# DakeQQ/Voice-Activity-Detection-VAD-ONNX

Measured on NVIDIA B200. Metric: RTFx (audio-hours/sec), higher is better.
Workload: dtype f32

## Files before the change

### include/vadx.h

```cpp
#ifndef VADX_H_
#define VADX_H_

#include <stddef.h>
#include <stdint.h>

#ifdef __cplusplus
extern "C" {
#endif

#define VADX_ABI_VERSION 1

enum {
  VADX_OK = 0,
  VADX_EINVAL = -1,
  VADX_ENODEVICE = -2,
  VADX_ECUDA = -3,
  VADX_EMISSING = -4,
  VADX_ENOMEM = -5
};

enum { VADX_DT_I16 = 0, VADX_DT_F32 = 1, VADX_DT_I32 = 2 };
enum { VADX_ACT_NONE = 0, VADX_ACT_RELU = 1, VADX_ACT_SIGMOID = 2, VADX_ACT_SOFTMAX = 3,
       VADX_ACT_LOG = 4, VADX_ACT_LOG_CLAMP = 5, VADX_ACT_RES_FIRST = 16 };
enum { VADX_FLOOR_CLAMP = 0, VADX_FLOOR_ADD = 1 };
enum { VADX_PREEMPH_NONE = 0, VADX_PREEMPH_ZERO_HISTORY = 1, VADX_PREEMPH_KEEP_FIRST = 2 };

int vadx_abi_version(void);
const char* vadx_last_error(void);
int vadx_device_count(void);
uint64_t vadx_launch_count(void);

enum {
  VADX_STAGE_PREP = 0,
  VADX_STAGE_STFT = 1,
  VADX_STAGE_MEL = 2,
  VADX_STAGE_LINEAR = 3,
  VADX_STAGE_MEMORY = 4,
  VADX_STAGE_HEAD = 5,
  VADX_STAGE_POSTPROC = 6,
  VADX_STAGE_COUNT = 7
};
int vadx_profile_enable(int on);
int vadx_profile_collect(double* ms, uint64_t* calls, int n_stages);
typedef struct vadx_kernel_stat {
  const char* name;
  double ms;
  uint64_t calls;
  double bytes;
  double flops;
} vadx_kernel_stat;
int vadx_profile_collect_kernels(vadx_kernel_stat* out, int capacity, int* n_out);


int vadx_prep_audio(const void* d_audio, int in_dtype, int64_t n_streams, int64_t n_samples,
                    int64_t in_stride, float scale, int remove_dc, int preemph_mode, float preemph,
                    int64_t pad_left, float* d_out, int64_t out_stride, void* stream);

int vadx_stft_power_f32(const float* d_sig, int64_t sig_stride, int64_t n_streams, int n_frames, int hop,
                        int n_taps, const float* d_basis, int ld_basis, int n_bins, float* d_power,
                        int64_t ld_power, void* stream);

int vadx_stft_tc_supported(int n_taps, int n_bins);
int vadx_pack_stft_basis_tc(const float* h_basis, int ld_basis, int n_taps, int n_bins, double preemph, double scale,
                            void* h_img, size_t img_capacity, size_t* img_bytes);
int vadx_stft_power_tc_i16(const int16_t* d_audio, int64_t in_stride, int64_t n_samples, int64_t n_streams,
                           int n_frames, int hop, int n_taps, const void* d_img, int n_bins, float* d_power,
                           int64_t ld_power, void* stream);
int vadx_pack_stft_dc_tc(const float* h_basis, int ld_basis, int n_taps, int n_bins, double preemph, double scale,
                         int64_t n_samples, int hop, int pad_left, int n_frames, float* h_tables, size_t capacity_floats,
                         size_t* n_floats, int* n_edge_lo, int* t_edge_hi);
int vadx_stream_mean_i16(const int16_t* d_audio, int64_t in_stride, int64_t n_samples, int64_t n_streams,
                         float* d_mean_frac, int32_t* d_mean_int, void* stream);
int vadx_stft_power_tc_i16_ex(const int16_t* d_audio, int64_t in_stride, int64_t n_samples, int64_t n_streams,
                              int n_frames, int hop, int n_taps, const void* d_img, int n_bins, float* d_power,
                              int64_t ld_power, int pad_left, const float* d_mean_frac, const int32_t* d_mean_int,
                              const float* d_dc_tables, int n_edge_lo, int t_edge_hi, float power_scale,
                              int operand_format, void* stream);
enum { VADX_TC_FMT_BF16 = 0, VADX_TC_FMT_F16 = 1 };
int vadx_pack_stft_basis_tc_fmt(const float* h_basis, int ld_basis, int n_taps, int n_bins, double preemph, double scale,
                                int operand_format, void* h_img, size_t img_capacity, size_t* img_bytes);

int vadx_mel_log_f32(const float* d_power, int64_t ld_power, int64_t n_rows, int n_bins, int n_mels,
                     const int32_t* d_start, const int32_t* d_len, const float* d_w, int max_len,
                     int floor_mode, float floor_value, float* d_out, int64_t ld_out, void* stream);

int vadx_linear_f32(const float* d_x, int64_t ldx, const float* d_wt, int ldw, const float* d_bias,
                    const float* d_residual, int64_t ldr, float* d_y, int64_t ldy, int64_t n_rows, int n_in,
                    int n_out, int act, void* stream);

int vadx_tc_supported(int n_in, int n_out);
int vadx_pack_weight_tc(const float* h_w, int n_out, int n_in, void* h_img, size_t img_capacity, size_t* img_bytes);
int vadx_linear_tc_f32(const float* d_x, int64_t ldx, const void* d_wimg, const float* d_bias,
                       const float* d_residual, int64_t ldr, float* d_y, int64_t ldy, int64_t n_rows, int n_in,
                       int n_out, int act, void* stream);

int vadx_depthwise_conv1d_f32(const float* d_x, int64_t ldx, const float* d_w, int kernel, int stride, int dilation,
                              int pad, float* d_y, int64_t ldy, int64_t n_streams, int t_in, int t_out,
                              int n_channels, void* stream);

int vadx_linear_head_tc_f32(const float* d_x, int64_t ldx, const void* d_wimg, const float* d_bias, int64_t n_rows,
                            int n_in, int n_out, int act, const float* d_head_w, float head_bias, float* d_head_out,
                            void* stream);

int vadx_fsmn_memory_f32(const float* d_p, int64_t ldp, const float* d_wl, int n_back, int stride_back,
                         const float* d_wr, int n_ahead, int stride_ahead, const float* d_residual,
                         int64_t ldr, float* d_out, int64_t ldo, int64_t n_streams, int n_frames,
                         int n_channels, const float* d_cache_in, float* d_cache_out, void* stream);

size_t vadx_fc2_memory_stages_stream_bytes(int n_in, int n_frames);
int vadx_fc2_memory_stages_supported(int n_in, int n_out, int n_frames, int n_back, int stride_back, int n_ahead,
                                     int stride_ahead);
int vadx_linear_tc_stream_stages_f32(const float* d_x, const void* d_wimg, const float* d_bias, void* d_himg,
                                     int64_t n_rows, int rows_per_stream, int n_in, int n_out, int act, void* stream);
int vadx_fc2_memory_stages_f32(const void* d_himg, int n_in, const void* d_wimg, const float* d_bias, int act,
                               const float* d_wl, int n_back, const float* d_wr, int n_ahead, const float* d_residual,
                               float* d_out, int64_t n_streams, int n_frames, void* stream);

int vadx_lfr_cmvn_f32(const float* d_mel, int64_t ld_mel, const float* d_mean, const float* d_var, float* d_out,
                      int64_t ld_out, int64_t n_streams, int n_frames, int n_mels, int lfr_m, int lfr_n, void* stream);

int vadx_softmax_class0_f32(const float* d_logits, int64_t ld, int64_t n_rows, int n_classes, float* d_p0,
                            void* stream);

int vadx_frame_energy_log10_f32(const float* d_sig, int64_t sig_stride, int64_t offset, int64_t n_streams, int win,
                                int hop, int n_energy, int n_frames, float scale, float eps, float* d_out,
                                void* stream);

int vadx_fsmn_gate(const float* d_p_sil, const float* d_power_dB, const float* d_noise_avg,
                   float one_minus_speech_threshold, float speech_2_noise_ratio, int64_t n_streams, int n_frames,
                   uint8_t* d_score, float* d_noisy_dB, void* stream);

int vadx_lookahead_hysteresis(const void* d_in, int mode, int64_t ld_in, int64_t n_streams, int n_frames,
                              int look_backward, double speaking_score, double silence_score, int is_final,
                              uint8_t* d_silence_state, int32_t* d_n_saved, uint8_t* d_saved, int64_t ld_saved,
                              float* d_noise_avg, const float* d_noisy_dB, float snr_threshold, void* stream);

int vadx_fsmn_gate_hysteresis_windows(const float* d_p_sil, const float* d_power_dB, int64_t n_streams, int n_windows,
                                      int n_frames, float one_minus_speech_threshold, float speech_2_noise_ratio,
                                      int look_backward, double speaking_score, double silence_score, uint8_t* d_score,
                                      float* d_noisy_dB, float* d_noise_in, uint8_t* d_silence_state, int32_t* d_n_saved,
                                      uint8_t* d_saved, int64_t ld_saved, float* d_noise_avg, float snr_threshold,
                                      void* stream);

int vadx_gather_windows_i16(const int16_t* d_in, int64_t stream_stride, int64_t n_streams, int n_windows, int64_t window_stride,
                            int64_t n_samples, int16_t* d_out, void* stream);

int vadx_runs_to_segments(const uint8_t* d_silence_flags, int64_t ld, const int32_t* d_n_flags, int64_t n_streams,
                          int32_t* d_seg_count, int32_t* d_segments, int max_segments, void* stream);

int vadx_stft_mag_compact_f32(const float* d_y, int64_t ldy, int64_t n_windows, int rows_per_window, int n_frames,
                              int n_bins, float* d_mag, void* stream);
int vadx_reflect_window_f32(const float* d_x, int64_t in_stride, int64_t n_streams, int n_in, int pad, float* d_out,
                            void* stream);
int vadx_reflect_windows_f32(const float* d_x, int64_t in_stride, int64_t n_streams, int n_windows, int64_t window_step,
                             int n_in, int pad, float* d_out, void* stream);
int vadx_sqrt_inplace_f32(float* d_p, int64_t n, void* stream);
int vadx_affine_f32(const float* d_x, float a, float b, float* d_y, int64_t n, void* stream);
int vadx_lstm_cell_f32(const float* d_gates, const float* d_c_in, float* d_h_out, float* d_c_out, float* d_h_relu,
                       int64_t n_streams, int hidden, void* stream);

int vadx_silero_lstm_windows_f32(const float* d_gates_in, const float* d_wt_hh, int ldw, const float* d_state_in,
                                 float* d_state_out, const float* d_head_w, float head_bias, float* d_probs,
                                 int64_t n_streams, int n_windows, int hidden, void* stream);

int vadx_silero_timestamps(const float* d_probs, int64_t ld, const int32_t* d_n_windows, const int64_t* d_n_samples,
                           int64_t n_streams, double threshold, double neg_threshold, double min_speech_samples,
                           double max_speech_samples, double min_silence_samples,
                           double min_silence_samples_at_max_speech, int window, int use_max_poss_sil,
                           int32_t* d_seg_count, int64_t* d_segments, int max_segments, void* stream);

int vadx_stft_complex_f32(const float* d_sig, int64_t sig_stride, int64_t n_streams, int n_frames, int hop, int n_taps,
                          const float* d_basis, int ld_basis, int n_bins, float* d_out, int64_t ld_out, void* stream);
int vadx_permute4_f32(const float* d_in, float* d_out, int64_t n0, int64_t n1, int64_t n2, int64_t n3, int p0, int p1,
                      int p2, int p3, void* stream);
int vadx_layernorm_f32(const float* d_x, int64_t n_rows, int row_len, const float* d_w, const float* d_b, float eps,
                       float* d_out, void* stream);
int vadx_layernorm_perm_f32(const float* d_x, int64_t n_rows, int n1, int n2, int n3, int q0, int q1, int q2, const float* d_w,
                            const float* d_b, int w_out_order, float eps, float* d_out, int64_t out_stride, int pad, void* stream);
int vadx_ceps_cmul_t_f32(const float* d_q, const float* d_spec, float* d_out, int64_t n_blocks, int n_channels, int n_ceps,
                         void* stream);
int vadx_add_transposed_f32(const float* d_a, int64_t a_block_stride, const float* d_t, float* d_out, int64_t n_blocks, int n_bins,
                            int n_channels, void* stream);
int vadx_cfb_front_supported(int n_in, int n_channels, int n_bins);
int vadx_cfb_front_f32(const float* d_x, int64_t n_blocks, int n_bins, int n_in, int n_channels, const float* d_ln0_w,
                       const float* d_ln0_b, const float* d_wg, const float* d_bg, const float* d_wi, const float* d_bi,
                       const float* d_ln1_w, const float* d_ln1_b, const float* d_ln2_w, const float* d_ln2_b, float eps,
                       float* d_col, float* d_z, void* stream);
int vadx_lstm_seq_f32(const float* d_x, int64_t x_outer, int64_t x_inner, int64_t x_step, float* d_y, int64_t y_outer,
                      int64_t y_inner, int64_t y_step, const float* d_w_ih, const float* d_w_hh, const float* d_b_ih,
                      const float* d_b_hh, int64_t n_seq, int n_inner, int seq_len, int n_in, int hidden, int reverse,
                      void* stream);
int vadx_lstm_recurrence_supported(int hidden);
int vadx_lstm_recurrence_f32(const float* d_gates_in, int64_t g_outer, int64_t g_inner, int64_t g_step, float* d_y,
                             int64_t y_outer, int64_t y_inner, int64_t y_step, const float* d_w_hh_perm, int64_t n_seq,
                             int n_inner, int seq_len, int hidden, int reverse, void* stream);
int vadx_ew2_f32(int op, const float* d_a, int64_t lda, const float* d_b, int64_t ldb, float* d_out, int64_t ldo,
                 float* d_out2, int64_t ldo2, int64_t n_rows, int n_cols, float scalar, void* stream);
int vadx_ceps_cmul_f32(const float* d_q, const float* d_p, float* d_out, int64_t n_rows, int n_channels, void* stream);
int vadx_im2col_f3_f32(const float* d_x, float* d_out, int64_t n_blocks, int n_bins, int n_channels, void* stream);
int vadx_alpha_x4_f32(const float* d_near_ri, const float* d_far_ri, int64_t n_streams, int n_frames, int n_bins, int k,
                      float w1_far, float w1_mix, float b1, const float* d_w2, float b2, float* d_x4, float* d_alpha,
                      void* stream);
int vadx_alpha_x4_const_f32(const float* d_near_ri, const float* d_pow_far, const float* d_far_comp, int t_max,
                            int64_t n_streams, int n_frames, int n_bins, int k, float w1_far, float w1_mix, float b1,
                            const float* d_w2, float b2, float* d_x4, float* d_alpha, void* stream);
int vadx_istft_ola_f32(const float* d_frames, int64_t ld, int64_t n_streams, int n_frames, int n_fft, int hop,
                       const float* d_wsum_inv, int n_out, float* d_y, int64_t ldy, void* stream);

int64_t vadx_ingest_out_frames(int64_t n_frames_in, int in_rate, int out_rate);
int vadx_ingest_pcm16(const int16_t* d_pcm, int64_t in_stride, const int64_t* d_n_in, int64_t n_streams,
                      int64_t n_frames_in, int n_channels, int in_rate, int out_rate, int16_t* d_out,
                      int64_t out_stride, int64_t* d_n_out, void* stream);

int64_t vadx_resample_out_len(int64_t n_in, double scale);
int vadx_resample_linear_f32(const float* d_in, int64_t in_stride, int64_t n_in, int64_t n_streams, double scale,
                             float* d_out, int64_t out_stride, int64_t out_offset, void* stream);

typedef struct {
  int32_t smooth_window;
  float threshold;
  int32_t min_speech_frame;
  int32_t max_speech_frame;
  int32_t min_silence_frame;
  int32_t merge_silence_frame;
  int32_t extend_speech_frame;
} vadx_post_cfg;
int vadx_postprocess_frames(const float* d_probs, int64_t ld_probs, const int32_t* d_n_frames,
                            int64_t n_streams, int n_frames, const vadx_post_cfg* cfg, int8_t* d_decisions,
                            int32_t* d_seg_count, int32_t* d_segments, int max_segments, void* stream);

typedef struct {
  int32_t smooth_window;
  float threshold;
  int32_t pad_start_frame;
  int32_t min_speech_frame;
  int32_t max_speech_frame;
  int32_t min_silence_frame;
} vadx_stream_post_cfg;
int vadx_stream_post_state_words(int smooth_window);
int vadx_stream_postprocess(const float* d_probs, int64_t ld_probs, const int32_t* d_n_frames, int64_t n_streams,
                            int n_frames, const vadx_stream_post_cfg* cfg, int32_t* d_state, int32_t* d_seg_count,
                            int32_t* d_segments, int max_segments, int32_t* d_open, void* stream);

#define VADX_SERVE_START 0
#define VADX_SERVE_END 1
#define VADX_SERVE_END_OF_STREAM 2
#define VADX_SERVE_ERR_RANGE 1
#define VADX_SERVE_ERR_SHORT 2
int vadx_stream_serve_zero_tail(int16_t* d_chunk, int64_t ld_chunk, const int32_t* d_n_samples, int64_t n_slots,
                                int chunk_samples, int frame_len, void* stream);
int vadx_stream_serve_step(const float* d_probs, int64_t ld_probs, int n_frames, const int32_t* d_n_samples,
                           const uint8_t* d_last, int64_t n_slots, int chunk_samples, int frame_len, int frame_hop,
                           const vadx_stream_post_cfg* cfg, int32_t* d_state, const float* d_caches_in,
                           float* d_caches_out, int n_cache_blocks, int64_t cache_row, int32_t* d_frames,
                           int32_t* d_events, int32_t* d_header, int32_t* h_events, int32_t* h_header, void* d_scratch,
                           size_t scratch_bytes, size_t* scratch_needed, void* stream);

int vadx_silero_serve_load(const int16_t* d_chunk, const int32_t* d_n_samples, int64_t n_slots, int windows_per_tick,
                           float* d_x, void* stream);
int vadx_silero_serve_step(const float* d_probs, int64_t ld_probs, const int32_t* d_n_samples, const uint8_t* d_last,
                           int64_t n_slots, int windows_per_tick, double threshold, double min_silence_samples,
                           int32_t* d_state, float* d_x, const float* d_state_in, float* d_state_out,
                           int32_t* d_windows, int32_t* d_events, int32_t* d_header, int32_t* h_events,
                           int32_t* h_header, void* d_scratch, size_t scratch_bytes, size_t* scratch_needed,
                           void* stream);

typedef struct vadx_model vadx_model;

int vadx_create(const char* kind, const int32_t* hparams, int n_hparams, vadx_model** out);
void vadx_destroy(vadx_model* m);

int vadx_set_tensor(vadx_model* m, const char* name, const void* h_data, int dtype, const int64_t* dims,
                    int n_dims);
int vadx_set_scalar(vadx_model* m, const char* name, double value);

int vadx_workspace_bytes(const vadx_model* m, int64_t n_streams, int64_t n_samples, size_t* out_bytes);
int vadx_output_frames(const vadx_model* m, int64_t n_samples, int32_t* out_frames);

int vadx_forward(vadx_model* m, const void* const* d_inputs, void* const* d_outputs, void* const* d_state,
                 int64_t n_streams, int64_t n_samples, void* d_workspace, size_t workspace_bytes,
                 void* stream);

#ifdef __cplusplus
}
#endif
#endif
```

### voice-activity-detection-vad-onnx_b200/csrc/model.cu

```cuda
#include "model.hpp"

struct FireRedHP : FrontendGeom {
  int idim, R, M, H, P, N1, S1, N2, S2, odim;
  int frames(int64_t L) const { return L < n_taps() ? 0 : (int)(1 + (L - n_taps()) / hop); }
};

static int firered_hp(const vadx_model* m, FireRedHP* h) {
  VADX_REQUIRE(m->hp.size() == 14, "firered: expected 14 hyper-parameters, got %zu", m->hp.size());
  const int32_t* v = m->hp.data();
  *h = FireRedHP{{v[10], v[11], v[12], v[13]}, v[0], v[1], v[2], v[3], v[4], v[5], v[6], v[7], v[8], v[9]};
  VADX_REQUIRE(h->idim == h->n_mels, "firered: idim (%d) must equal n_mels (%d)", h->idim, h->n_mels);
  VADX_REQUIRE(h->R >= 1 && h->M >= 1 && h->H >= 1 && h->P >= 1 && h->N1 >= 1 && h->S1 >= 1 && h->N2 >= 0 &&
                   h->odim >= 1 && h->odim <= 8 && h->hop >= 1 && h->n_fft >= 2,
               "firered: hyper-parameter out of range");
  return VADX_OK;
}

static Frontend firered_frontend(const vadx_model* m, const FireRedHP& h) {
  return Frontend{h, (int)m->scalar("derived.bins_used", (double)h.n_bins()), 0, 1.0f, false, VADX_PREEMPH_ZERO_HISTORY,
                  VADX_TC_FMT_F16, VADX_FLOOR_CLAMP, (float)m->scalar("frontend.log_floor", 1e-7), frontend_rate_scale(m),
                  false};
}

int firered_finalize(vadx_model* m) {
  FireRedHP h;
  VADX_TRY(firered_hp(m, &h));
  int bins_used = 1;
  {
    const HostTensor* ms = m->find("frontend.mel_start");
    const HostTensor* ml = m->find("frontend.mel_len");
    if (ms && ml && ms->dtype == VADX_DT_I32 && ml->dtype == VADX_DT_I32 && ms->numel() == h.n_mels && ml->numel() == h.n_mels) {
      const int32_t* a = reinterpret_cast<const int32_t*>(ms->bytes.data());
      const int32_t* b = reinterpret_cast<const int32_t*>(ml->bytes.data());
      for (int i = 0; i < h.n_mels; ++i) bins_used = std::max(bins_used, a[i] + b[i]);
    } else {
      bins_used = h.n_bins();
    }
    bins_used = std::min(bins_used, h.n_bins());
    m->scalars["derived.bins_used"] = bins_used;
  }
  VADX_TRY(firered_frontend(m, h).finalize(m));
  VADX_TRY(m->upload_linear("dfsmn.fc1.0.weight", h.H, h.idim));
  VADX_TRY(m->upload_raw("dfsmn.fc1.0.bias", h.H, VADX_DT_F32));
  VADX_TRY(m->upload_linear("dfsmn.fc2.0.weight", h.P, h.H));
  VADX_TRY(m->upload_raw("dfsmn.fc2.0.bias", h.P, VADX_DT_F32));
  auto memory = [&](const std::string& pre) -> int {
    VADX_TRY(m->upload_raw(pre + "lookback_filter.weight", (int64_t)h.P * h.N1, VADX_DT_F32));
    if (h.N2 > 0) VADX_TRY(m->upload_raw(pre + "lookahead_filter.weight", (int64_t)h.P * h.N2, VADX_DT_F32));
    return VADX_OK;
  };
  VADX_TRY(memory("dfsmn.fsmn1."));
  for (int i = 0; i < h.R - 1; ++i) {
    std::string pre = "dfsmn.fsmns." + std::to_string(i) + ".";
    VADX_TRY(m->upload_linear(pre + "fc1.0.weight", h.H, h.P));
    VADX_TRY(m->upload_raw(pre + "fc1.0.bias", h.H, VADX_DT_F32));
    VADX_TRY(m->upload_linear(pre + "fc2.weight", h.P, h.H));
    VADX_TRY(memory(pre + "fsmn."));
  }
  VADX_TRY(m->upload_linear("dfsmn.dnns.0.weight", h.H, h.P));
  VADX_TRY(m->upload_raw("dfsmn.dnns.0.bias", h.H, VADX_DT_F32));
  for (int j = 1; j < h.M; ++j) {
    std::string n = "dfsmn.dnns." + std::to_string(2 * j);
    VADX_TRY(m->upload_linear(n + ".weight", h.H, h.H));
    VADX_TRY(m->upload_raw(n + ".bias", h.H, VADX_DT_F32));
  }
  VADX_TRY(m->upload_linear("out.weight", h.odim, h.H));
  VADX_TRY(m->upload_raw("out.weight", (int64_t)h.odim * h.H, VADX_DT_F32));
  VADX_TRY(m->upload_raw("out.bias", h.odim, VADX_DT_F32));
  return VADX_OK;
}

int firered_check(const vadx_model* m) {
  FireRedHP h;
  return firered_hp(m, &h);
}
int firered_frames(const vadx_model* m, int64_t n_samples, int32_t* out) {
  FireRedHP h;
  VADX_TRY(firered_hp(m, &h));
  const double sc = frontend_rate_scale(m);
  *out = h.frames(sc == 1.0 ? n_samples : vadx_resample_out_len(n_samples, sc));
  return VADX_OK;
}

static int64_t firered_slab(const vadx_model* m, int64_t S) {
  int64_t slab = (int64_t)m->scalar("engine.slab_streams", 0.0);
  if (slab <= 0 || slab > S) slab = S;
  return slab;
}

int firered_run(vadx_model* m, bool dry, const void* const* in, void* const* out, void* const* state, int64_t S_all,
                int64_t L, void* ws_ptr, size_t ws_bytes, size_t* need, cudaStream_t st) {
  FireRedHP h;
  VADX_TRY(firered_hp(m, &h));
  const int16_t* d_audio_all = dry ? nullptr : static_cast<const int16_t*>(in[0]);
  float* d_probs_all = dry ? nullptr : static_cast<float*>(out[0]);
  const float* cin_all = (!dry && state && state[0]) ? static_cast<const float*>(state[0]) : nullptr;
  float* cout_all = (!dry && state && state[0]) ? static_cast<float*>(state[1]) : nullptr;
  if (cin_all) {
    VADX_REQUIRE(h.N2 == 0, "firered: the streaming graph has no look-ahead taps (N2 must be 0, got %d)", h.N2);
    VADX_REQUIRE(cout_all && cout_all != cin_all, "firered: streaming needs a caches_out buffer distinct from caches_in");
  }
  const int64_t cache_stream = (int64_t)h.P * (h.N1 - 1) * h.S1;
  const int64_t cache_layer = S_all * cache_stream;
  const Frontend fe = firered_frontend(m, h);
  const double rate_scale = fe.rate_scale;
  const int64_t L16 = rate_scale == 1.0 ? L : vadx_resample_out_len(L, rate_scale);
  const int T = h.frames(L16);
  VADX_REQUIRE(T >= 1, "firered: %lld samples are shorter than one %d-sample frame", (long long)L16, h.n_taps());
  const int64_t slab = firered_slab(m, S_all);
  const int64_t slab_rows = slab * T;
  const int64_t Lp = round_up(std::max(L, L16), 4);
  Workspace ws(ws_ptr, ws_bytes, dry);
  float* sig = ws.take<float>(slab * Lp);
  float* sig2 = rate_scale == 1.0 ? nullptr : ws.take<float>(slab * Lp);
  float* power = ws.take<float>(slab_rows * h.ld_power());
  float* feat = ws.take<float>(slab_rows * h.n_mels);
  const int64_t bufH_floats = std::max<int64_t>(round_up(slab_rows, 128) * h.H,
                                                (h.H % 64) == 0 ? slab * (int64_t)(fc2_memory_stages_stream_bytes(h.H, T) / 4) : 0);
  float* bufH = ws.take<float>(bufH_floats);
  float* bufH2 = h.M > 1 ? ws.take<float>(slab_rows * h.H) : nullptr;
  float* bufP = ws.take<float>(slab_rows * h.P);
  float* memA0 = ws.take<float>(slab_rows * h.P);
  float* memB0 = ws.take<float>(slab_rows * h.P);
  if (need) *need = ws.off;
  if (dry) return VADX_OK;
  if (ws.off > ws_bytes) {
    set_error("firered: workspace of %zu bytes is smaller than the %zu needed", ws_bytes, ws.off);
    return VADX_ENOMEM;
  }

  for (int64_t s0 = 0; s0 < S_all; s0 += slab) {
    const int64_t S = std::min(slab, S_all - s0);
    const int64_t rows = S * T;
    const int16_t* d_audio = d_audio_all + s0 * L;
    float* d_probs = d_probs_all + s0 * (int64_t)h.odim * T;
    const float* cin = cin_all ? cin_all + s0 * cache_stream : nullptr;
    float* cout = cin_all ? cout_all + s0 * cache_stream : nullptr;
    float* memA = memA0;
    float* memB = memB0;
    const bool use_tc = m->scalar("engine.use_tc", 1.0) != 0.0 && rows > kSkinnyMaxRows;
    VADX_TRY(fe.run(m, d_audio, S, L, T, FrontendBufs{sig, sig2, Lp, power, nullptr, nullptr, feat}, st));
    auto lin = [&](const float* x, int n_in, const std::string& w, const char* b, const float* res, float* y, int n_out,
                   int act) -> int {
      const uint8_t* img = use_tc ? m->d<uint8_t>(w + "#TC") : nullptr;
      if (img)
        return vadx_linear_tc_f32(x, n_in, img, b ? m->d<float>(b) : nullptr, res, n_out, y, n_out, rows, n_in, n_out,
                                  act, st);
      return vadx_linear_f32(x, n_in, m->d<float>(w + "#T"), (int)round_up(n_out, 4), b ? m->d<float>(b) : nullptr, res,
                             n_out, y, n_out, rows, n_in, n_out, act, st);
    };
    auto memory = [&](int layer, const std::string& pre, const float* p, const float* res, float* o) -> int {
      return vadx_fsmn_memory_f32(p, h.P, m->d<float>(pre + "lookback_filter.weight"), h.N1, h.S1,
                                  h.N2 > 0 ? m->d<float>(pre + "lookahead_filter.weight") : nullptr, h.N2,
                                  h.N2 > 0 ? h.S2 : 1, res, h.P, o, h.P, S, T, h.P,
                                  cin ? cin + layer * cache_layer : nullptr, cin ? cout + layer * cache_layer : nullptr,
                                  st);
    };
    const bool split_hidden = use_tc && (h.H % 64) == 0 && m->scalar("engine.split_hidden", 1.0) != 0.0;
    const bool fuse_stages = split_hidden && !cin && fc2_memory_stages_supported(h.H, h.P, T, h.N1, h.S1, h.N2, h.N2 > 0 ? h.S2 : 1) &&
                             m->scalar("engine.fuse_stages", 1.0) != 0.0 &&
                             S * (int64_t)fc2_memory_stages_stream_bytes(h.H, T) < (1LL << 32);
    auto fc1 = [&](const float* x, int n_in, const std::string& w, const char* b) -> int {
      if (fuse_stages)
        return linear_tc_stream_stages_f32(x, m->d<uint8_t>(w + "#TC"), b ? m->d<float>(b) : nullptr, bufH, rows, T, n_in, h.H,
                                           VADX_ACT_RELU, st);
      const uint8_t* img = split_hidden ? m->d<uint8_t>(w + "#TC") : nullptr;
      if (img) return linear_tc_stages_f32(x, img, b ? m->d<float>(b) : nullptr, bufH, rows, n_in, h.H, VADX_ACT_RELU, 0, 1, st);
      return lin(x, n_in, w, b, nullptr, bufH, h.H, VADX_ACT_RELU);
    };
    auto block_tail = [&](const std::string& w, const char* b, int act, const std::string& mem_pre, int layer, const float* res,
                          float* o) -> int {
      if (fuse_stages)
        return fc2_memory_stages_f32(bufH, h.H, m->d<uint8_t>(w + "#TC"), b ? m->d<float>(b) : nullptr, act,
                                     m->d<float>(mem_pre + "lookback_filter.weight"), h.N1,
                                     m->d<float>(mem_pre + "lookahead_filter.weight"), h.N2, res, o, S, T, st);
      const uint8_t* simg = split_hidden ? m->d<uint8_t>(w + "#TC") : nullptr;
      if (simg) VADX_TRY(linear_tc_stages_f32(bufH, simg, b ? m->d<float>(b) : nullptr, bufP, rows, h.H, h.P, act, 1, 0, st));
      else VADX_TRY(lin(bufH, h.H, w, b, nullptr, bufP, h.P, act));
      return memory(layer, mem_pre, bufP, res, o);
    };
    VADX_TRY(fc1(feat, h.idim, "dfsmn.fc1.0.weight", "dfsmn.fc1.0.bias"));
    VADX_TRY(block_tail("dfsmn.fc2.0.weight", "dfsmn.fc2.0.bias", VADX_ACT_RELU, "dfsmn.fsmn1.", 0, nullptr, memA));
    for (int i = 0; i < h.R - 1; ++i) {
      std::string pre = "dfsmn.fsmns." + std::to_string(i) + ".";
      std::string b1 = pre + "fc1.0.bias";
      VADX_TRY(fc1(memA, h.P, pre + "fc1.0.weight", b1.c_str()));
      VADX_TRY(block_tail(pre + "fc2.weight", nullptr, VADX_ACT_NONE, pre + "fsmn.", i + 1, memA, memB));
      std::swap(memA, memB);
    }
    if (use_tc && h.M == 1 && h.odim == 1 && m->d<uint8_t>("dfsmn.dnns.0.weight#TC")) {
      const HostTensor* ob = m->find("out.bias");
      VADX_TRY(vadx_linear_head_tc_f32(memA, h.P, m->d<uint8_t>("dfsmn.dnns.0.weight#TC"),
                                       m->d<float>("dfsmn.dnns.0.bias"), rows, h.P, h.H, VADX_ACT_RELU,
                                       m->d<float>("out.weight"), ob->f32()[0], d_probs, st));
      continue;
    }
    VADX_TRY(lin(memA, h.P, "dfsmn.dnns.0.weight", "dfsmn.dnns.0.bias", nullptr, bufH, h.H, VADX_ACT_RELU));
    float* hcur = bufH;
    float* hnext = bufH2;
    for (int j = 1; j < h.M; ++j) {
      std::string n = "dfsmn.dnns." + std::to_string(2 * j);
      std::string b = n + ".bias";
      VADX_TRY(lin(hcur, h.H, n + ".weight", b.c_str(), nullptr, hnext, h.H, VADX_ACT_RELU));
      std::swap(hcur, hnext);
    }
    VADX_TRY(linear_narrow(hcur, h.H, m->d<float>("out.weight#T"), (int)round_up(h.odim, 4), m->d<float>("out.bias"),
                           d_probs, rows, h.H, h.odim, VADX_ACT_SIGMOID, T, (int64_t)h.odim * T, T, st));
  }
  return VADX_OK;
}

namespace {
struct KindOps {
  const char* name;
  int (*check)(const vadx_model*);
  int (*finalize)(vadx_model*);
  int (*frames)(const vadx_model*, int64_t, int32_t*);
  int (*run)(vadx_model*, bool, const void* const*, void* const*, void* const*, int64_t, int64_t, void*, size_t,
             size_t*, cudaStream_t);
};
const KindOps kKinds[] = {
    {"firered", firered_check, firered_finalize, firered_frames, firered_run},
    {"fsmn", fsmn_check, fsmn_finalize, fsmn_frames, fsmn_run},
    {"silero", silero_check, silero_finalize, silero_frames, silero_run},
    {"marblenet", marblenet_check, marblenet_finalize, marblenet_frames, marblenet_run},
    {"dfsmn_aec", dfsmn_check, dfsmn_finalize, dfsmn_frames, dfsmn_run},
};
const KindOps* ops_of(const std::string& kind) {
  for (const auto& k : kKinds)
    if (kind == k.name) return &k;
  return nullptr;
}
}

extern "C" int vadx_create(const char* kind, const int32_t* hparams, int n_hparams, vadx_model** out) {
  VADX_REQUIRE(kind && out && (n_hparams == 0 || hparams), "vadx_create: null pointer");
  const KindOps* ops = ops_of(kind);
  VADX_REQUIRE(ops, "vadx_create: unknown model kind '%s'", kind);
  if (vadx_device_count() < 1) {
    set_error("vadx_create: no CUDA device is visible; libvadx has no CPU path");
    return VADX_ENODEVICE;
  }
  vadx_model* m = new vadx_model();
  m->kind = kind;
  m->hp.assign(hparams, hparams + n_hparams);
  int rc = ops->check(m);
  if (rc != VADX_OK) {
    delete m;
    return rc;
  }
  *out = m;
  return VADX_OK;
}

extern "C" void vadx_destroy(vadx_model* m) { delete m; }

extern "C" int vadx_set_tensor(vadx_model* m, const char* name, const void* h_data, int dtype, const int64_t* dims,
                               int n_dims) {
  VADX_REQUIRE(m && name && h_data && dims && n_dims >= 1 && n_dims <= 8, "vadx_set_tensor: bad argument");
  VADX_REQUIRE(dtype == VADX_DT_I16 || dtype == VADX_DT_F32 || dtype == VADX_DT_I32, "vadx_set_tensor: dtype %d", dtype);
  HostTensor t;
  t.dtype = dtype;
  t.dims.assign(dims, dims + n_dims);
  for (int i = 0; i < n_dims; ++i) VADX_REQUIRE(dims[i] >= 0, "vadx_set_tensor: negative dim");
  size_t esz = dtype == VADX_DT_I16 ? 2 : 4;
  t.bytes.resize((size_t)t.numel() * esz);
  memcpy(t.bytes.data(), h_data, t.bytes.size());
  m->host[name] = std::move(t);
  m->finalized = false;
  return VADX_OK;
}

extern "C" int vadx_set_scalar(vadx_model* m, const char* name, double value) {
  VADX_REQUIRE(m && name, "vadx_set_scalar: null pointer");
  if (!strncmp(name, "frontend.", 9)) m->finalized = false;
  m->scalars[name] = value;
  return VADX_OK;
}

extern "C" int vadx_output_frames(const vadx_model* m, int64_t n_samples, int32_t* out_frames) {
  VADX_REQUIRE(m && out_frames, "vadx_output_frames: null pointer");
  return ops_of(m->kind)->frames(m, n_samples, out_frames);
}

extern "C" int vadx_workspace_bytes(const vadx_model* m, int64_t n_streams, int64_t n_samples, size_t* out_bytes) {
  VADX_REQUIRE(m && out_bytes && n_streams >= 0 && n_samples >= 0, "vadx_workspace_bytes: bad argument");
  return ops_of(m->kind)->run(const_cast<vadx_model*>(m), true, nullptr, nullptr, nullptr, n_streams, n_samples,
                              nullptr, 0, out_bytes, nullptr);
}

extern "C" int vadx_forward(vadx_model* m, const void* const* d_inputs, void* const* d_outputs, void* const* d_state,
                            int64_t n_streams, int64_t n_samples, void* d_workspace, size_t workspace_bytes,
                            void* stream) {
  VADX_REQUIRE(m && d_inputs && d_outputs && d_inputs[0] && d_outputs[0], "vadx_forward: null pointer");
  VADX_REQUIRE(n_streams >= 0 && n_samples > 0, "vadx_forward: bad shape S=%lld L=%lld", (long long)n_streams,
               (long long)n_samples);
  VADX_REQUIRE(d_workspace || workspace_bytes == 0, "vadx_forward: null workspace");
  const KindOps* ops = ops_of(m->kind);
  if (!m->finalized) {
    m->release();
    VADX_TRY(ops->finalize(m));
    m->finalized = true;
  }
  if (n_streams == 0) return VADX_OK;
  return ops->run(m, false, d_inputs, d_outputs, d_state, n_streams, n_samples, d_workspace, workspace_bytes, nullptr,
                  (cudaStream_t)stream);
}
```

### voice-activity-detection-vad-onnx_b200/csrc/model.hpp

```cpp
#pragma once
#include <algorithm>
#include <cstring>
#include <map>
#include <string>
#include <vector>

#include "common.cuh"

namespace vadx {
int linear_narrow(const float* d_x, int64_t ldx, const float* d_wt, int ldw, const float* d_bias, float* d_y,
                  int64_t n_rows, int n_in, int n_out, int act, int rows_per_group, int64_t group_stride,
                  int64_t out_stride, cudaStream_t st);

struct HostTensor {
  std::vector<char> bytes;
  std::vector<int64_t> dims;
  int dtype = VADX_DT_F32;
  int64_t numel() const {
    int64_t n = 1;
    for (auto d : dims) n *= d;
    return n;
  }
  const float* f32() const { return reinterpret_cast<const float*>(bytes.data()); }
};

struct DevBuf {
  void* p = nullptr;
  size_t bytes = 0;
};

struct Workspace {
  char* base;
  size_t cap, off = 0;
  bool dry;
  Workspace(void* b, size_t c, bool d) : base((char*)b), cap(c), dry(d) {}
  template <typename T>
  T* take(int64_t n) {
    size_t bytes = (size_t)round_up((int64_t)(n * sizeof(T)), 256);
    char* p = dry ? nullptr : base + off;
    off += bytes;
    return reinterpret_cast<T*>(p);
  }
};

}

int linear_tc_stages_f32(const float* d_x, const void* d_wimg, const float* d_bias, float* d_y, int64_t n_rows, int n_in,
                         int n_out, int act, int x_split, int y_split, void* stream);

int linear_tc_stream_stages_f32(const float* d_x, const void* d_wimg, const float* d_bias, float* d_y, int64_t n_rows,
                                int rows_per_stream, int n_in, int n_out, int act, void* stream);
size_t fc2_memory_stages_stream_bytes(int n_in, int n_frames);
bool fc2_memory_stages_supported(int n_in, int n_out, int n_frames, int n_back, int stride_back, int n_ahead, int stride_ahead);
int fc2_memory_stages_f32(const void* d_himg, int n_in, const void* d_wimg, const float* d_bias, int act, const float* d_wl,
                          int n_back, const float* d_wr, int n_ahead, const float* d_res, float* d_out, int64_t n_streams,
                          int n_frames, void* stream);

using namespace vadx;

struct vadx_model {
  std::string kind;
  std::vector<int32_t> hp;
  std::map<std::string, HostTensor> host;
  std::map<std::string, double> scalars;
  std::map<std::string, DevBuf> dev;
  bool finalized = false;

  ~vadx_model() { release(); }
  void release() {
    for (auto& kv : dev)
      if (kv.second.p) cudaFree(kv.second.p);
    dev.clear();
    finalized = false;
  }
  double scalar(const char* name, double dflt) const {
    auto it = scalars.find(name);
    return it == scalars.end() ? dflt : it->second;
  }
  const HostTensor* find(const std::string& n) const {
    auto it = host.find(n);
    return it == host.end() ? nullptr : &it->second;
  }
    int upload(const std::string& key, const void* src, size_t bytes) {
    DevBuf b;
    b.bytes = bytes;
    cudaError_t e = cudaMalloc(&b.p, std::max<size_t>(bytes, 16));
    if (e != cudaSuccess) return cuda_fail(e, "cudaMalloc(constant)");
    e = cudaMemcpy(b.p, src, bytes, cudaMemcpyHostToDevice);
    if (e != cudaSuccess) {
      cudaFree(b.p);
      return cuda_fail(e, "cudaMemcpy(constant)");
    }
    auto it = dev.find(key);
    if (it != dev.end() && it->second.p) cudaFree(it->second.p);
    dev[key] = b;
    return VADX_OK;
  }
  int upload_linear(const std::string& name, int n_out, int n_in) {
    const HostTensor* t = find(name);
    if (!t) {
      set_error("model '%s': tensor '%s' was never set", kind.c_str(), name.c_str());
      return VADX_EMISSING;
    }
    if (t->dtype != VADX_DT_F32 || t->numel() != (int64_t)n_out * n_in) {
      set_error("tensor '%s': expected %d x %d fp32, got %lld elements", name.c_str(), n_out, n_in,
                (long long)t->numel());
      return VADX_EINVAL;
    }
    int ldw = (int)round_up(n_out, 4);
    std::vector<float> wt((size_t)n_in * ldw, 0.f);
    const float* w = t->f32();
    for (int o = 0; o < n_out; ++o)
      for (int i = 0; i < n_in; ++i) wt[(size_t)i * ldw + o] = w[(size_t)o * n_in + i];
    VADX_TRY(upload(name + "#T", wt.data(), wt.size() * sizeof(float)));
    bool placed = false;
    if (vadx_tc_supported(n_in, n_out)) {
      size_t bytes = 0;
      VADX_TRY(vadx_pack_weight_tc(w, n_out, n_in, nullptr, 0, &bytes));
      std::vector<uint8_t> img(bytes);
      VADX_TRY(vadx_pack_weight_tc(w, n_out, n_in, img.data(), img.size(), &bytes));
      VADX_TRY(upload(name + "#TC", img.data(), img.size()));
      placed = true;
    } else if (n_in > 256 && n_out > 8 && n_out <= 256) {
      const int n_parts = (n_in + 255) / 256;
      const int pk = (int)round_up((n_in + n_parts - 1) / n_parts, 64);
      if (vadx_tc_supported(pk, n_out) && n_in - (n_parts - 1) * pk > 0) {
        for (int part = 0; part < n_parts; ++part) {
          const int k0 = part * pk, kn = std::min(pk, n_in - k0);
          std::vector<float> sub((size_t)n_out * kn);
          for (int o = 0; o < n_out; ++o)
            for (int i = 0; i < kn; ++i) sub[(size_t)o * kn + i] = w[(size_t)o * n_in + k0 + i];
          size_t bytes = 0;
          VADX_TRY(vadx_pack_weight_tc(sub.data(), n_out, kn, nullptr, 0, &bytes));
          std::vector<uint8_t> img(bytes);
          VADX_TRY(vadx_pack_weight_tc(sub.data(), n_out, kn, img.data(), img.size(), &bytes));
          VADX_TRY(upload(name + "#TCK" + std::to_string(part), img.data(), img.size()));
        }
        scalars["derived.ksplit." + name] = pk;
        placed = true;
      }
    }
    if (!placed && n_out > 16) {
      for (int wmax : {256, 128, 64}) {
        const int n_blocks = (n_out + wmax - 1) / wmax;
        const int bw = (int)round_up((n_out + n_blocks - 1) / n_blocks, 16);
        if (n_blocks < 2 || !vadx_tc_supported(n_in, bw) || n_out - (n_blocks - 1) * bw <= 8) continue;
        for (int j = 0; j < n_blocks; ++j) {
          const int c0 = j * bw, cn = std::min(bw, n_out - c0);
          size_t bytes = 0;
          VADX_TRY(vadx_pack_weight_tc(w + (size_t)c0 * n_in, cn, n_in, nullptr, 0, &bytes));
          std::vector<uint8_t> img(bytes);
          VADX_TRY(vadx_pack_weight_tc(w + (size_t)c0 * n_in, cn, n_in, img.data(), img.size(), &bytes));
          VADX_TRY(upload(name + "#TCN" + std::to_string(j), img.data(), img.size()));
        }
        scalars["derived.nsplit." + name] = bw;
        break;
      }
    }
    return VADX_OK;
  }
  int linear(const std::string& name, const float* x, int64_t ldx, const float* bias, const float* res, int64_t ldr, float* y,
             int64_t ldy, int64_t n_rows, int n_in, int n_out, int act, bool use_tc, void* st) const {
    if (use_tc && n_rows > kSkinnyMaxRows) {
      if (const uint8_t* img = d<uint8_t>(name + "#TC"))
        return vadx_linear_tc_f32(x, ldx, img, bias, res, ldr, y, ldy, n_rows, n_in, n_out, act, st);
      const int pk = (int)scalar(("derived.ksplit." + name).c_str(), 0.0);
      if (pk > 0 && !res && (act & VADX_ACT_RES_FIRST) == 0) {
        for (int part = 0, k0 = 0; k0 < n_in; ++part, k0 += pk) {
          const bool first = part == 0, last = k0 + pk >= n_in;
          VADX_TRY(vadx_linear_tc_f32(x + k0, ldx, d<uint8_t>(name + "#TCK" + std::to_string(part)), first ? bias : nullptr,
                                      first ? nullptr : y, ldy, y, ldy, n_rows, std::min(pk, n_in - k0), n_out,
                                      last ? (act | (first ? 0 : VADX_ACT_RES_FIRST)) : VADX_ACT_NONE, st));
        }
        return VADX_OK;
      }
      const int bw = (int)scalar(("derived.nsplit." + name).c_str(), 0.0);
      if (bw > 0 && ((ldy & 3) == 0 || (bw & 3) == 0)) {
        for (int j = 0, c0 = 0; c0 < n_out; ++j, c0 += bw)
          VADX_TRY(vadx_linear_tc_f32(x, ldx, d<uint8_t>(name + "#TCN" + std::to_string(j)), bias ? bias + c0 : nullptr,
                                      res ? res + c0 : nullptr, ldr, y + c0, ldy, n_rows, n_in, std::min(bw, n_out - c0), act, st));
        return VADX_OK;
      }
    }
    return vadx_linear_f32(x, ldx, d<float>(name + "#T"), (int)round_up(n_out, 4), bias, res, ldr, y, ldy, n_rows, n_in, n_out,
                           act, st);
  }
  int upload_mel_dense_tc(int n_mels, int n_bins, float floor_value) {
    const HostTensor* ms = find("frontend.mel_start");
    const HostTensor* ml = find("frontend.mel_len");
    const HostTensor* mw = find("frontend.mel_w");
    if (!ms || !ml || !mw || ms->numel() != n_mels || ml->numel() != n_mels || !vadx_tc_supported(n_bins, n_mels)) return VADX_OK;
    const int max_len = (int)(mw->numel() / n_mels);
    const int32_t* a = reinterpret_cast<const int32_t*>(ms->bytes.data());
    const int32_t* b = reinterpret_cast<const int32_t*>(ml->bytes.data());
    std::vector<float> dense((size_t)n_mels * n_bins, 0.f);
    for (int i = 0; i < n_mels; ++i)
      for (int j = 0; j < b[i] && a[i] + j < n_bins; ++j) dense[(size_t)i * n_bins + a[i] + j] = mw->f32()[(size_t)i * max_len + j];
    size_t bytes = 0;
    VADX_TRY(vadx_pack_weight_tc(dense.data(), n_mels, n_bins, nullptr, 0, &bytes));
    std::vector<uint8_t> img(bytes);
    VADX_TRY(vadx_pack_weight_tc(dense.data(), n_mels, n_bins, img.data(), img.size(), &bytes));
    VADX_TRY(upload("frontend.mel#TC", img.data(), img.size()));
    std::vector<float> fl((size_t)n_mels, floor_value);
    return upload("frontend.mel_floor", fl.data(), fl.size() * sizeof(float));
  }
  int upload_raw(const std::string& name, int64_t expect_numel, int dtype) {
    const HostTensor* t = find(name);
    if (!t) {
      set_error("model '%s': tensor '%s' was never set", kind.c_str(), name.c_str());
      return VADX_EMISSING;
    }
    if (t->dtype != dtype || (expect_numel >= 0 && t->numel() != expect_numel)) {
      set_error("tensor '%s': expected %lld elements of dtype %d, got %lld of dtype %d", name.c_str(),
                (long long)expect_numel, dtype, (long long)t->numel(), t->dtype);
      return VADX_EINVAL;
    }
    return upload(name, t->bytes.data(), t->bytes.size());
  }
  template <typename T>
  const T* d(const std::string& key) const {
    auto it = dev.find(key);
    return it == dev.end() ? nullptr : reinterpret_cast<const T*>(it->second.p);
  }
  bool has(const std::string& n) const { return host.count(n) != 0; }
};


struct FrontendGeom {
  int n_fft, win, hop, n_mels;
  int n_taps() const { return win < n_fft ? win : n_fft; }
  int first_tap() const { return win < n_fft ? (n_fft - win) / 2 : 0; }
  int n_bins() const { return n_fft / 2 + 1; }
  int ld_basis() const { return (int)round_up(2 * n_bins(), 4); }
  int ld_power() const { return (int)round_up(n_bins(), 4); }
  int pad_left() const { return n_fft / 2 - first_tap(); }
};

struct FrontendBufs {
  float* sig;
  float* sig2;
  int64_t Lp;
  float* power;
  float* mean;
  int32_t* mean_int;
  float* mel;
};

struct Frontend {
  FrontendGeom g;
  int n_bins;
  int pad_left;
  float in_scale;
  bool remove_dc;
  int preemph_mode;
  int tc_format;
  int floor_mode;
  float floor_value;
  double rate_scale;
  bool keep_signal;

  int finalize(vadx_model* m) const;
  int run(vadx_model* m, const int16_t* audio, int64_t S, int64_t L, int T, const FrontendBufs& b, cudaStream_t st) const;
};

inline double frontend_rate_scale(const vadx_model* m) {
  const double in_rate = m->scalar("frontend.in_sample_rate", 16000.0);
  return in_rate == 16000.0 ? 1.0 : 1.0 / (in_rate / 16000.0);
}

inline int Frontend::finalize(vadx_model* m) const {
  VADX_TRY(m->upload_raw("frontend.basis", (int64_t)g.n_taps() * g.ld_basis(), VADX_DT_F32));
  if (vadx_stft_tc_supported(g.n_taps(), n_bins)) {
    const double preemph = m->scalar("frontend.preemph", 0.97);
    const float* hb = m->find("frontend.basis")->f32();
    size_t bytes = 0;
    VADX_TRY(vadx_pack_stft_basis_tc_fmt(hb, g.ld_basis(), g.n_taps(), n_bins, preemph, 1.0, tc_format, nullptr, 0, &bytes));
    std::vector<uint8_t> img(bytes);
    VADX_TRY(vadx_pack_stft_basis_tc_fmt(hb, g.ld_basis(), g.n_taps(), n_bins, preemph, 1.0, tc_format, img.data(), img.size(),
                                         &bytes));
    VADX_TRY(m->upload("frontend.basis#TC", img.data(), img.size()));
  }
  VADX_TRY(m->upload_raw("frontend.mel_start", g.n_mels, VADX_DT_I32));
  VADX_TRY(m->upload_raw("frontend.mel_len", g.n_mels, VADX_DT_I32));
  VADX_TRY(m->upload_raw("frontend.mel_w", -1, VADX_DT_F32));
  return m->upload_mel_dense_tc(g.n_mels, n_bins, floor_value);
}

inline int Frontend::run(vadx_model* m, const int16_t* audio, int64_t S, int64_t L, int T, const FrontendBufs& b,
                         cudaStream_t st) const {
  const int64_t rows = S * T;
  const bool use_tc = m->scalar("engine.use_tc", 1.0) != 0.0 && rows > kSkinnyMaxRows;
  const float preemph = (float)m->scalar("frontend.preemph", 0.97);
  const int pre = preemph > 0.f ? preemph_mode : 0;
  const int64_t Lp = b.Lp;
  const uint8_t* stft_img = use_tc ? m->d<uint8_t>("frontend.basis#TC") : nullptr;
  if (rate_scale != 1.0) {
    if (rate_scale < 1.0) {
      VADX_TRY(vadx_prep_audio(audio, VADX_DT_I16, S, L, L, 1.0f, 0, 0, 0.f, 0, b.sig2, Lp, st));
      VADX_TRY(vadx_resample_linear_f32(b.sig2, Lp, L, S, rate_scale, b.sig, Lp, 0, st));
      VADX_TRY(vadx_prep_audio(b.sig, VADX_DT_F32, S, vadx_resample_out_len(L, rate_scale), Lp, in_scale, remove_dc, pre,
                               preemph, pad_left, b.sig2, Lp, st));
    } else {
      VADX_TRY(vadx_prep_audio(audio, VADX_DT_I16, S, L, L, in_scale, remove_dc, pre, preemph, 0, b.sig, Lp, st));
      if (pad_left > 0) {
        cudaError_t e = cudaMemsetAsync(b.sig2, 0, (size_t)S * Lp * sizeof(float), st);
        if (e != cudaSuccess) return cuda_fail(e, "cudaMemsetAsync(frontend centre pad)");
      }
      VADX_TRY(vadx_resample_linear_f32(b.sig, Lp, L, S, rate_scale, b.sig2, Lp, pad_left, st));
    }
    VADX_TRY(vadx_stft_power_f32(b.sig2, Lp, S, T, g.hop, g.n_taps(), m->d<float>("frontend.basis"), g.ld_basis(), n_bins,
                                 b.power, g.ld_power(), st));
  } else {
    const bool tc = stft_img && (L % 8) == 0 && (g.hop % 16) == 0 && (pad_left % 8) == 0 && aligned16(audio);
    if (keep_signal || !tc)
      VADX_TRY(vadx_prep_audio(audio, VADX_DT_I16, S, L, L, in_scale, remove_dc, pre, preemph, pad_left, b.sig, Lp, st));
    if (tc) {
      const float* dc = nullptr;
      int lo = 0, hi = T;
      if (remove_dc || pad_left > 0) {
        const std::string key = "frontend.dc#" + std::to_string((long long)L);
        const std::string k_lo = key + ".lo", k_hi = key + ".hi";
        if (!m->d<float>(key)) {
          size_t n = 0;
          const float* hb = m->find("frontend.basis")->f32();
          VADX_TRY(vadx_pack_stft_dc_tc(hb, g.ld_basis(), g.n_taps(), n_bins, preemph, 1.0, L, g.hop, pad_left, T, nullptr, 0,
                                        &n, &lo, &hi));
          std::vector<float> tab(n);
          VADX_TRY(vadx_pack_stft_dc_tc(hb, g.ld_basis(), g.n_taps(), n_bins, preemph, 1.0, L, g.hop, pad_left, T, tab.data(),
                                        tab.size(), &n, &lo, &hi));
          VADX_TRY(m->upload(key, tab.data(), tab.size() * sizeof(float)));
          m->scalars[k_lo] = lo;
          m->scalars[k_hi] = hi;
        }
        dc = m->d<float>(key);
        lo = (int)m->scalar(k_lo.c_str(), 0.0);
        hi = (int)m->scalar(k_hi.c_str(), (double)T);
      }
      if (remove_dc) VADX_TRY(vadx_stream_mean_i16(audio, L, L, S, b.mean, b.mean_int, st));
      VADX_TRY(vadx_stft_power_tc_i16_ex(audio, L, L, S, T, g.hop, g.n_taps(), stft_img, n_bins, b.power, g.ld_power(), pad_left,
                                         remove_dc ? b.mean : nullptr, remove_dc ? b.mean_int : nullptr, dc, lo, hi,
                                         in_scale * in_scale, tc_format, st));
    } else {
      VADX_TRY(vadx_stft_power_f32(b.sig, Lp, S, T, g.hop, g.n_taps(), m->d<float>("frontend.basis"), g.ld_basis(), n_bins,
                                   b.power, g.ld_power(), st));
    }
  }
  if (use_tc && m->d<uint8_t>("frontend.mel#TC")) {
    return vadx_linear_tc_f32(b.power, g.ld_power(), m->d<uint8_t>("frontend.mel#TC"), m->d<float>("frontend.mel_floor"),
                              nullptr, 0, b.mel, g.n_mels, rows, n_bins, g.n_mels,
                              floor_mode == VADX_FLOOR_CLAMP ? VADX_ACT_LOG_CLAMP : VADX_ACT_LOG, st);
  }
  const int mel_max = (int)(m->find("frontend.mel_w")->numel() / g.n_mels);
  return vadx_mel_log_f32(b.power, g.ld_power(), rows, n_bins, g.n_mels, m->d<int32_t>("frontend.mel_start"),
                          m->d<int32_t>("frontend.mel_len"), m->d<float>("frontend.mel_w"), mel_max, floor_mode, floor_value,
                          b.mel, g.n_mels, st);
}


int firered_check(const vadx_model* m);
int firered_finalize(vadx_model* m);
int firered_frames(const vadx_model* m, int64_t n_samples, int32_t* out);
int firered_run(vadx_model* m, bool dry, const void* const* in, void* const* out, void* const* state, int64_t S,
                int64_t L, void* ws_ptr, size_t ws_bytes, size_t* need, cudaStream_t st);
int marblenet_check(const vadx_model* m);
int marblenet_finalize(vadx_model* m);
int marblenet_frames(const vadx_model* m, int64_t n_samples, int32_t* out);
int marblenet_run(vadx_model* m, bool dry, const void* const* in, void* const* out, void* const* state, int64_t S,
                  int64_t L, void* ws_ptr, size_t ws_bytes, size_t* need, cudaStream_t st);
int silero_check(const vadx_model* m);
int silero_finalize(vadx_model* m);
int silero_frames(const vadx_model* m, int64_t n_samples, int32_t* out);
int silero_run(vadx_model* m, bool dry, const void* const* in, void* const* out, void* const* state, int64_t S,
               int64_t L, void* ws_ptr, size_t ws_bytes, size_t* need, cudaStream_t st);
int fsmn_check(const vadx_model* m);
int fsmn_finalize(vadx_model* m);
int fsmn_frames(const vadx_model* m, int64_t n_samples, int32_t* out);
int fsmn_run(vadx_model* m, bool dry, const void* const* in, void* const* out, void* const* state, int64_t S,
             int64_t L, void* ws_ptr, size_t ws_bytes, size_t* need, cudaStream_t st);
int dfsmn_check(const vadx_model* m);
int dfsmn_finalize(vadx_model* m);
int dfsmn_frames(const vadx_model* m, int64_t n_samples, int32_t* out);
int dfsmn_run(vadx_model* m, bool dry, const void* const* in, void* const* out, void* const* state, int64_t S, int64_t L,
              void* ws_ptr, size_t ws_bytes, size_t* need, cudaStream_t st);
```

### voice-activity-detection-vad-onnx_b200/csrc/stft_tc.cu

```cuda
#include "tc_ptx.cuh"

namespace vadx {

constexpr int kStNPad = 80;
constexpr int kStTerms = 2;
constexpr int kStLead = 8;
constexpr int kStJ = 2;
constexpr int kStSlices = 2 * kStJ;
constexpr int kStStages = 3;
constexpr int kStLoaderWarps = 16;
constexpr int kStOutLd = 44;

struct StftTcArgs {
  const int16_t* X;
  int64_t in_stride;
  int64_t L;
  int64_t S;
  int n_frames, hop;
  int h16;
  int n_q;
  int tq;
  int rows;
  int slice_units;
  int n_st;
  const uint8_t* Wimg;
  float* P;
  int64_t ldp;
  int n_bins, kc, n_k16, n_tiles, vec_p;
  int pad_left;
  const float* mean;
  const int* mean_int;
  const float* dc;
  int n_edge_lo, t_edge_hi;
  float power_scale;
  int stage_out;
  unsigned backoff_ld, backoff_epi;
  int debug;
};

__device__ __forceinline__ uint32_t bf16x2_lo(uint32_t w) {
  const float a = __uint_as_float(0x4B000000u | (w & 0xffu)) - 8388608.0f;
  const float b = __uint_as_float(0x4B000000u | ((w >> 16) & 0xffu)) - 8388608.0f;
  return __byte_perm(__float_as_uint(a), __float_as_uint(b), 0x7632);
}
__device__ __forceinline__ uint32_t bf16x2_hi(uint32_t w) {
  const uint32_t ha = (((w >> 8) & 0xffu) ^ 0x80u);
  const uint32_t hb = (((w >> 24) & 0xffu) ^ 0x80u);
  const float a = fmaf(__uint_as_float(0x4B000000u | ha), 256.0f, -(8388608.0f + 128.0f) * 256.0f);
  const float b = fmaf(__uint_as_float(0x4B000000u | hb), 256.0f, -(8388608.0f + 128.0f) * 256.0f);
  return __byte_perm(__float_as_uint(a), __float_as_uint(b), 0x7632);
}

__device__ __forceinline__ uint32_t f16x2_lo(uint32_t w) {
  const uint32_t m = (w & 0x00ff00ffu) | 0x64006400u;
  uint32_t r;
  asm("sub.rn.f16x2 %0, %1, %2;" : "=r"(r) : "r"(m), "r"(0x64006400u));
  return r;
}
__device__ __forceinline__ uint32_t f16x2_hi(uint32_t w) {
  const uint32_t m = (((w >> 8) & 0x00ff00ffu) ^ 0x00800080u) | 0x64006400u;
  uint32_t r;
  asm("sub.rn.f16x2 %0, %1, %2;" : "=r"(r) : "r"(m), "r"(0x64806480u));
  asm("mul.rn.f16x2 %0, %1, %2;" : "=r"(r) : "r"(r), "r"(0x5c005c00u));
  return r;
}

__device__ __forceinline__ void split17(int d, float& hi, float& lo) {
  lo = __uint_as_float(0x4B000000u | (uint32_t)(d & 255)) - 8388608.0f;
  const uint32_t h = (uint32_t)((d >> 8) + 256);
  hi = fmaf(__uint_as_float(0x4B000000u | h), 256.0f, -(8388608.0f + 256.0f) * 256.0f);
}

template <bool EX, bool F16>
__global__ void __launch_bounds__((kStLoaderWarps + 5) * 32, 1) stft_power_tc_kernel(const StftTcArgs g) {
  constexpr int kStEpiWarp0 = kStLoaderWarps, kStMmaWarp = kStLoaderWarps + 4;
  extern __shared__ __align__(1024) uint8_t smem_raw[];
  uint8_t* w_smem = smem_raw;
  const uint32_t img_bytes = kStNPad * 128u;
  const int w_bytes = g.kc * kStTerms * (int)img_bytes;
  uint8_t* a_smem = w_smem + w_bytes;
  const uint32_t slice_bytes = (uint32_t)g.slice_units * 16u;
  const uint32_t term_bytes = kStSlices * slice_bytes;
  const uint32_t stage_bytes = 2u * term_bytes;
  uint64_t* bars = reinterpret_cast<uint64_t*>(a_smem + (size_t)kStStages * stage_bytes);
  uint32_t* tmem_slot = reinterpret_cast<uint32_t*>(bars + 13);
  float* out_stage = reinterpret_cast<float*>(bars + 16);

  const int warp = threadIdx.x >> 5, lane = threadIdx.x & 31;
  const uint32_t bar0 = smem_u32(bars);
  auto full_bar = [&](int s) { return bar0 + 8u * s; };
  auto empty_bar = [&](int s) { return bar0 + 8u * (4 + s); };
  auto tfull_bar = [&](int b) { return bar0 + 8u * (8 + b); };
  auto tempty_bar = [&](int b) { return bar0 + 8u * (10 + b); };
  const uint32_t wbar = bar0 + 8u * 12;
  constexpr int kAccN = 2 * kStNPad;
  constexpr uint32_t kTmemCols = 512;

  if (threadIdx.x == 0) {
    for (int s = 0; s < kStStages; ++s) {
      mbar_init(full_bar(s), kStLoaderWarps);
      mbar_init(empty_bar(s), 1);
    }
    for (int b = 0; b < 2; ++b) {
      mbar_init(tfull_bar(b), 1);
      mbar_init(tempty_bar(b), 4);
    }
    mbar_init(wbar, 1);
    asm volatile("fence.mbarrier_init.release.cluster;" ::: "memory");
  }
  if (warp == kStMmaWarp) {
    asm volatile("tcgen05.alloc.cta_group::1.sync.aligned.shared::cta.b32 [%0], %1;" ::"r"(smem_u32(tmem_slot)),
                 "r"(kTmemCols)
                 : "memory");
    asm volatile("tcgen05.relinquish_alloc_permit.cta_group::1.sync.aligned;" ::: "memory");
  }
  tc_fence_before();
  __syncthreads();
  tc_fence_after();
  const uint32_t tmem_base = *tmem_slot;
  const int ntile = blockIdx.y;

  if (warp == kStMmaWarp) {
    if (lane == 0) {
      mbar_expect_tx(wbar, (uint32_t)w_bytes);
      const uint8_t* src = g.Wimg + (size_t)ntile * w_bytes;
      for (int t = 0; t < g.kc * kStTerms; ++t) bulk_g2s(smem_u32(w_smem) + t * img_bytes, src + (size_t)t * img_bytes, img_bytes, wbar);
      mbar_wait(wbar, 0);
      const uint32_t idesc = F16 ? umma_idesc_f16(kAccN) : umma_idesc_bf16(kAccN);
      const uint64_t dw = umma_desc_sw128(smem_u32(w_smem));
      const uint64_t da0 = umma_desc_noswz(smem_u32(a_smem), slice_bytes, 128u);
      const uint32_t chunk_units = (kStTerms * img_bytes) >> 4, lo_units = term_bytes >> 4, stage_units = stage_bytes >> 4;
      const uint32_t col_units = (2u * slice_bytes) >> 4;
      const int h16 = g.h16, n_k16 = g.n_k16;
      const uint32_t lo_on = (g.debug & 4) ? 0u : 1u;
      constexpr bool kBurst = F16 && !EX;
      auto b_desc = [&](int k) { return dw + (uint64_t)((uint32_t)(k >> 2) * chunk_units + 2u * (uint32_t)(k & 3)); };
      int stage = 0;
      uint32_t phase = 0;
      int it = 0;
      for (int tile = blockIdx.x; tile < g.n_tiles; tile += gridDim.x, ++it) {
        const int b = it & 1;
        const uint32_t use = (uint32_t)(it >> 1);
        mbar_wait(tempty_bar(b), (use & 1u) ^ 1u);
        tc_fence_after();
        const uint32_t d_tmem = tmem_base + (uint32_t)(b * kAccN);
        for (int st = 0; st < g.n_st; ++st) {
          mbar_wait(full_bar(stage), phase);
          tc_fence_after();
          const uint64_t da_st = da0 + (uint64_t)stage * stage_units;
#pragma unroll
          for (int jj = 0; jj < kStJ; ++jj) {
            const int j = st * kStJ + jj;
            if (j >= h16) break;
            const uint64_t da_j = da_st + (uint64_t)jj * col_units;
            if (kBurst) {
              for (int q0 = 0, k = j; k < n_k16; q0 += 3, k += 3 * h16) {
                const int n_pairs = 1 + (k + h16 < n_k16 ? 1 : 0) + (k + 2 * h16 < n_k16 ? 1 : 0);
                umma_split_x3(d_tmem, da_j + (uint64_t)q0, 1u, lo_units, b_desc(k), b_desc(k + h16), b_desc(k + 2 * h16),
                              idesc, k ? 1u : 0u, n_pairs, lo_on);
              }
            } else {
              for (int q = 0, k = j; k < n_k16; ++q, k += h16) {
                const uint64_t da = da_j + (uint64_t)q;
                if (g.debug & 4) umma_bf16(d_tmem, da, b_desc(k), idesc, k ? 1u : 0u);
                else umma_x2(d_tmem, da, da + lo_units, b_desc(k), idesc, k ? 1u : 0u);
              }
            }
          }
          umma_commit(empty_bar(stage));
          if (++stage == kStStages) { stage = 0; phase ^= 1u; }
        }
        umma_commit(tfull_bar(b));
      }
    }
  } else if (warp < kStLoaderWarps) {
    constexpr int kRowsPerPass = kStLoaderWarps * 32 / kStSlices;
    constexpr int kPasses = 2;
    const int t = threadIdx.x;
    const int sl = t % kStSlices;
    const int r_in = t / kStSlices;
    const int16_t* xs_n[kPasses];
    int h0_n[kPasses];
    uint32_t rok_n = 0u;
    int tile_cached = -1;
    struct Seq { int tile, st; };
    auto valid = [&](const Seq& q) { return q.tile < g.n_tiles; };
    auto advance = [&](Seq& q) { if (++q.st == g.n_st) { q.st = 0; q.tile += gridDim.x; } };
    const int n_groups = 2 * g.h16;
    auto issue = [&](const Seq& q, uint4* raw, uint32_t& msk) {
      msk = 0u;
      if (q.tile != tile_cached) {
        rok_n = 0u;
#pragma unroll
        for (int pass = 0; pass < kPasses; ++pass) {
          const int r = pass * kRowsPerPass + r_in;
          const int64_t slot = (int64_t)q.tile * kTcBM + r;
          const int64_t s = slot / g.tq;
          const int h = (int)(slot - s * g.tq);
          const bool ok = r < g.rows && s < g.S;
          xs_n[pass] = g.X + (ok ? s : 0) * g.in_stride;
          h0_n[pass] = h * g.hop - (EX ? g.pad_left : 0) - kStLead;
          if (ok) rok_n |= 1u << pass;
        }
        tile_cached = q.tile;
      }
      const int grp = q.st * kStSlices + sl;
#pragma unroll
      for (int pass = 0; pass < kPasses; ++pass) {
        const int i0 = h0_n[pass] + 8 * grp;
        uint4 v = make_uint4(0u, 0u, 0u, 0u);
        if (((rok_n >> pass) & 1u) && grp < n_groups && i0 >= 0 && i0 + 7 < g.L) {
          v = __ldg(reinterpret_cast<const uint4*>(xs_n[pass] + i0));
          msk |= 1u << pass;
        }
        raw[pass] = v;
      }
    };
    int stage = 0;
    uint32_t phase = 0;
    int mi_c[kPasses];
#pragma unroll
    for (int pass = 0; pass < kPasses; ++pass) mi_c[pass] = 0;
    int tile_cached_c = -1;
    auto consume = [&](const Seq& q, const uint4* raw, uint32_t msk) {
      if (EX && g.mean_int && q.tile != tile_cached_c) {
#pragma unroll
        for (int pass = 0; pass < kPasses; ++pass) {
          const int64_t s = ((int64_t)q.tile * kTcBM + pass * kRowsPerPass + r_in) / g.tq;
          mi_c[pass] = s < g.S ? __ldg(g.mean_int + s) : 0;
        }
        tile_cached_c = q.tile;
      }
      mbar_wait(empty_bar(stage), phase ^ 1u, g.backoff_ld);
      uint8_t* st_hi = a_smem + (size_t)stage * stage_bytes + sl * slice_bytes;
      uint8_t* st_lo = st_hi + term_bytes;
      if (!(g.debug & 8) && q.st * kStSlices + sl < n_groups)
#pragma unroll
      for (int pass = 0; pass < kPasses; ++pass) {
        const int r = pass * kRowsPerPass + r_in;
        if (r >= g.rows) break;
        const uint32_t wds[4] = {raw[pass].x, raw[pass].y, raw[pass].z, raw[pass].w};
        uint32_t hi[4], lo[4];
        if (EX && g.mean_int) {
          const int mi = ((msk >> pass) & 1u) ? mi_c[pass] : 0;
#pragma unroll
          for (int j = 0; j < 4; ++j) {
            const uint32_t w = wds[j];
            const int a = ((int)(w << 16) >> 16) - mi;
            const int b = ((int)w >> 16) - mi;
            float ah, al, bh, bl;
            split17(a, ah, al);
            split17(b, bh, bl);
            hi[j] = __byte_perm(__float_as_uint(ah), __float_as_uint(bh), 0x7632);
            lo[j] = __byte_perm(__float_as_uint(al), __float_as_uint(bl), 0x7632);
          }
        } else {
#pragma unroll
        for (int j = 0; j < 4; ++j) {
          const uint32_t w = wds[j];
          hi[j] = F16 ? f16x2_hi(w) : bf16x2_hi(w);
          lo[j] = F16 ? f16x2_lo(w) : bf16x2_lo(w);
        }
        }
        *reinterpret_cast<uint4*>(st_hi + r * 16) = make_uint4(hi[0], hi[1], hi[2], hi[3]);
        *reinterpret_cast<uint4*>(st_lo + r * 16) = make_uint4(lo[0], lo[1], lo[2], lo[3]);
      }
      if (!(g.debug & 16)) fence_proxy_async();
      __syncwarp();
      if (lane == 0) mbar_arrive(full_bar(stage));
      if (++stage == kStStages) { stage = 0; phase ^= 1u; }
    };
    constexpr int kStBufs = EX ? 4 : 6;
    uint4 bufs[kStBufs][kPasses];
    uint32_t msks[kStBufs];
#pragma unroll
    for (int i = 0; i < kStBufs; ++i) msks[i] = 0u;
    Seq nxt{(int)blockIdx.x, 0}, cur{(int)blockIdx.x, 0};
#pragma unroll
    for (int i = 0; i < kStBufs - 1; ++i)
      if (valid(nxt)) { issue(nxt, bufs[i], msks[i]); advance(nxt); }
    while (valid(cur)) {
#pragma unroll
      for (int i = 0; i < kStBufs; ++i) {
        constexpr int kPrev = kStBufs - 1;
        if (valid(nxt)) { issue(nxt, bufs[(i + kPrev) % kStBufs], msks[(i + kPrev) % kStBufs]); advance(nxt); }
        consume(cur, bufs[i], msks[i]); advance(cur);
        if (!valid(cur)) break;
      }
    }
  } else {
    const int q = warp - kStEpiWarp0;
    int it = 0;
    const int f0 = ntile * (kStNPad / 2);
    for (int tile = blockIdx.x; tile < g.n_tiles; tile += gridDim.x, ++it) {
      const int b = it & 1;
      const uint32_t use = (uint32_t)(it >> 1);
      mbar_wait(tfull_bar(b), use & 1u, g.backoff_epi);
      tc_fence_after();
      const int64_t slot = (int64_t)tile * kTcBM + q * 32 + lane;
      const int64_t sidx = slot / g.tq;
      const int t = (int)(slot - sidx * g.tq);
      const bool row_ok = sidx < g.S && t < g.n_frames;
      const int64_t row = row_ok ? sidx * g.n_frames + t : -1;
      const uint32_t taddr = tmem_base + ((uint32_t)(q * 32) << 16) + (uint32_t)(b * kAccN);
      float* const my_out = out_stage + (size_t)q * 32 * kStOutLd;
      float m_row = 0.f, x_last = 0.f;
      const float* dc_row = nullptr;
      const float* tail_row = nullptr;
      if (EX && g.dc && row_ok) {
        const int n_edge = g.n_edge_lo + (g.n_frames - g.t_edge_hi);
        if (g.mean) {
          m_row = __ldg(g.mean + sidx);
          const int e = t < g.n_edge_lo ? 1 + t : (t >= g.t_edge_hi ? 1 + g.n_edge_lo + (t - g.t_edge_hi) : 0);
          dc_row = g.dc + ((size_t)e * gridDim.y + ntile) * kStNPad;
        }
        if (t >= g.t_edge_hi) {
          x_last = (float)((int)__ldg(g.X + sidx * g.in_stride + (g.L - 1)) - (g.mean_int ? __ldg(g.mean_int + sidx) : 0));
          tail_row = g.dc + ((size_t)(1 + n_edge + (t - g.t_edge_hi)) * gridDim.y + ntile) * kStNPad;
        }
      }
#pragma unroll
      for (int c0 = 0; c0 < kStNPad; c0 += 16) {
        float v[16], v2[16];
        tmem_ld16(taddr + (uint32_t)c0, v);
        tmem_ld16(taddr + (uint32_t)(kStNPad + c0), v2);
#pragma unroll
        for (int j = 0; j < 16; ++j) v[j] += v2[j];
        if (!row_ok || (g.debug & 1)) continue;
        if (EX && dc_row) {
#pragma unroll
          for (int j = 0; j < 16; ++j) v[j] = fmaf(-m_row, __ldg(dc_row + c0 + j), v[j]);
        }
        if (EX && tail_row) {
#pragma unroll
          for (int j = 0; j < 16; ++j) v[j] = fmaf(x_last, __ldg(tail_row + c0 + j), v[j]);
        }
        float* out = g.P + row * g.ldp + f0 + c0 / 2;
        float pw[8];
#pragma unroll
        for (int j = 0; j < 8; ++j) pw[j] = (v[2 * j] * v[2 * j] + v[2 * j + 1] * v[2 * j + 1]) * g.power_scale;
        const int fb = f0 + c0 / 2;
        if (g.stage_out) {
          float4* d4 = reinterpret_cast<float4*>(my_out + lane * kStOutLd + c0 / 2);
          d4[0] = make_float4(pw[0], pw[1], pw[2], pw[3]);
          d4[1] = make_float4(pw[4], pw[5], pw[6], pw[7]);
        } else if (g.vec_p && fb + 7 < g.n_bins) {
          reinterpret_cast<float4*>(out)[0] = make_float4(pw[0], pw[1], pw[2], pw[3]);
          reinterpret_cast<float4*>(out)[1] = make_float4(pw[4], pw[5], pw[6], pw[7]);
        } else {
#pragma unroll
          for (int j = 0; j < 8; ++j)
            if (fb + j < g.n_bins) out[j] = pw[j];
        }
      }
      tc_fence_before();
      __syncwarp();
      if (lane == 0) mbar_arrive(tempty_bar(b));
      if (g.stage_out && !(g.debug & 1)) {
        constexpr int kC4 = kStNPad / 8;
#pragma unroll
        for (int itr = 0; itr < kC4; ++itr) {
          const int idx = itr * 32 + lane;
          const int r = idx / kC4, c4 = idx - r * kC4;
          const long long grow = __shfl_sync(0xffffffffu, (long long)row, r);
          const int fbin = f0 + c4 * 4;
          if (grow >= 0 && fbin < g.n_bins) {
            const float4 val = *reinterpret_cast<const float4*>(my_out + r * kStOutLd + c4 * 4);
            float* out = g.P + grow * g.ldp + fbin;
            if (fbin + 3 < g.n_bins) {
              *reinterpret_cast<float4*>(out) = val;
            } else {
              out[0] = val.x;
              if (fbin + 1 < g.n_bins) out[1] = val.y;
              if (fbin + 2 < g.n_bins) out[2] = val.z;
            }
          }
        }
        __syncwarp();
      }
    }
  }
  tc_fence_before();
  __syncthreads();
  if (warp == kStMmaWarp) {
    tc_fence_after();
    asm volatile("tcgen05.dealloc.cta_group::1.sync.aligned.b32 %0, %1;" ::"r"(tmem_base), "r"(kTmemCols) : "memory");
  }
}

struct StftTcRing {
  int n_q, rows, slice_units;
  size_t bytes;
};
static StftTcRing stft_tc_ring(int n_k16, int h16) {
  StftTcRing r{};
  r.n_q = (n_k16 - 1) / h16 + 1;
  r.rows = kTcBM + r.n_q - 1;
  r.slice_units = r.rows + ((2 - r.rows % 4) + 4) % 4;
  r.bytes = (size_t)kStStages * 2 * kStSlices * r.slice_units * 16;
  return r;
}

struct StftTcShape {
  int kc, n_k16, n_ntiles;
  size_t tile_bytes, img_bytes, smem_bytes, stage_bytes;
  bool ok;
};
StftTcShape stft_tc_shape(int n_taps, int n_bins, int hop = 16) {
  StftTcShape s{};
  const int k_used = n_taps + kStLead;
  s.kc = (int)ceil_div(k_used, kTcBK);
  s.n_k16 = (int)ceil_div(k_used, 16);
  s.n_ntiles = (int)ceil_div(2 * n_bins, kStNPad);
  s.tile_bytes = (size_t)s.kc * kStTerms * kStNPad * 128;
  s.img_bytes = s.tile_bytes * s.n_ntiles;
  s.smem_bytes = s.tile_bytes + stft_tc_ring(s.n_k16, std::max(1, hop / 16)).bytes + 16 * 8;
  s.stage_bytes = (size_t)4 * 32 * kStOutLd * sizeof(float);
  s.ok = s.smem_bytes <= (size_t)kTcSmemBudget;
  return s;
}

}

using namespace vadx;

extern "C" int vadx_stft_tc_supported(int n_taps, int n_bins) { return stft_tc_shape(n_taps, n_bins).ok ? 1 : 0; }

extern "C" int vadx_pack_stft_basis_tc(const float* h_basis, int ld_basis, int n_taps, int n_bins, double preemph,
                                       double scale, void* h_img, size_t img_capacity, size_t* img_bytes) {
  return vadx_pack_stft_basis_tc_fmt(h_basis, ld_basis, n_taps, n_bins, preemph, scale, VADX_TC_FMT_BF16, h_img, img_capacity,
                                     img_bytes);
}

extern "C" int vadx_pack_stft_basis_tc_fmt(const float* h_basis, int ld_basis, int n_taps, int n_bins, double preemph,
                                           double scale, int operand_format, void* h_img, size_t img_capacity,
                                           size_t* img_bytes) {
  VADX_REQUIRE(h_basis && img_bytes && n_taps > 0 && n_bins > 0 && ld_basis >= 2 * n_bins,
               "vadx_pack_stft_basis_tc: bad argument");
  VADX_REQUIRE(operand_format == VADX_TC_FMT_BF16 || operand_format == VADX_TC_FMT_F16, "vadx_pack_stft_basis_tc: operand format %d",
               operand_format);
  const bool f16 = operand_format == VADX_TC_FMT_F16;
  StftTcShape s = stft_tc_shape(n_taps, n_bins);
  VADX_REQUIRE(s.ok, "vadx_pack_stft_basis_tc: %d taps x %d bins does not fit the tensor-core DFT", n_taps, n_bins);
  *img_bytes = s.img_bytes;
  if (!h_img) return VADX_OK;
  VADX_REQUIRE(img_capacity >= s.img_bytes, "vadx_pack_stft_basis_tc: image buffer too small");
  uint8_t* img = static_cast<uint8_t*>(h_img);
  memset(img, 0, s.img_bytes);
  const int n_cols = 2 * n_bins;
  const size_t term = (size_t)kStNPad * 128;
  for (int col = 0; col < n_cols; ++col) {
    const int nt = col / kStNPad, r = col % kStNPad;
    for (int k = 0; k < n_taps + kStLead; ++k) {
      const int n0 = k - kStLead, n1 = k - kStLead + 1;
      double v = 0.0;
      if (n0 >= 0 && n0 < n_taps) v += (double)h_basis[(size_t)n0 * ld_basis + col];
      if (n1 >= 0 && n1 < n_taps) v -= preemph * (double)h_basis[(size_t)n1 * ld_basis + col];
      v *= scale;
      const float f = (float)v;
      const uint16_t b0 = f16 ? f16_rn_host(f) : bf16_rn_host(f);
      const float r1 = (float)(v - (double)(f16 ? f16_to_f_host(b0) : bf16_to_f_host(b0)));
      const uint16_t b1 = f16 ? f16_rn_host(r1) : bf16_rn_host(r1);
      const int c = k / kTcBK, kk = k % kTcBK;
      uint8_t* base = img + (size_t)nt * s.tile_bytes + (size_t)(c * kStTerms) * term + sw128_offset(r, kk);
      memcpy(base, &b0, 2);
      memcpy(base + term, &b1, 2);
    }
  }
  return VADX_OK;
}

extern "C" int vadx_pack_stft_dc_tc(const float* h_basis, int ld_basis, int n_taps, int n_bins, double preemph, double scale,
                                    int64_t n_samples, int hop, int pad_left, int n_frames, float* h_tables,
                                    size_t capacity_floats, size_t* n_floats, int* n_edge_lo, int* t_edge_hi) {
  VADX_REQUIRE(h_basis && n_floats && n_edge_lo && t_edge_hi && n_taps > 0 && n_bins > 0 && hop > 0 && pad_left >= 0 &&
                   n_frames > 0 && ld_basis >= 2 * n_bins,
               "vadx_pack_stft_dc_tc: bad argument");
  StftTcShape s = stft_tc_shape(n_taps, n_bins);
  VADX_REQUIRE(s.ok, "vadx_pack_stft_dc_tc: shape not supported");
  int lo = 0;
  while (lo < n_frames && (int64_t)lo * hop - pad_left < 1) ++lo;
  int hi = n_frames;
  while (hi > lo && (int64_t)(hi - 1) * hop - pad_left + n_taps - 1 >= n_samples) --hi;
  *n_edge_lo = lo;
  *t_edge_hi = hi;
  const int n_edge = lo + (n_frames - hi);
  const size_t ncp = (size_t)s.n_ntiles * kStNPad;
  *n_floats = (size_t)(1 + n_edge + (n_frames - hi)) * ncp;
  if (!h_tables) return VADX_OK;
  VADX_REQUIRE(capacity_floats >= *n_floats, "vadx_pack_stft_dc_tc: table buffer too small");
  memset(h_tables, 0, *n_floats * sizeof(float));
  auto fill = [&](float* row, int64_t origin, bool interior) {
    for (int col = 0; col < 2 * n_bins; ++col) {
      double acc = 0.0;
      for (int n = 0; n < n_taps; ++n) {
        const int64_t i = origin + n;
        double coef = interior ? 1.0 - preemph : (i < 0 || i >= n_samples ? 0.0 : (i == 0 ? 1.0 : 1.0 - preemph));
        acc += coef * (double)h_basis[(size_t)n * ld_basis + col];
      }
      row[col] = (float)(acc * scale);
    }
  };
  fill(h_tables, 0, true);
  int e = 1;
  for (int t = 0; t < lo; ++t, ++e) fill(h_tables + (size_t)e * ncp, (int64_t)t * hop - pad_left, false);
  for (int t = hi; t < n_frames; ++t, ++e) fill(h_tables + (size_t)e * ncp, (int64_t)t * hop - pad_left, false);
  for (int t = hi; t < n_frames; ++t, ++e) {
    const int64_t n_l = n_samples - ((int64_t)t * hop - pad_left);
    if (n_l < 0 || n_l >= n_taps) continue;
    float* row = h_tables + (size_t)e * ncp;
    for (int col = 0; col < 2 * n_bins; ++col) row[col] = (float)(preemph * scale * (double)h_basis[(size_t)n_l * ld_basis + col]);
  }
  return VADX_OK;
}

namespace vadx {
__global__ void __launch_bounds__(256) stream_mean_i16_kernel(const int16_t* __restrict__ x, int64_t in_stride, int64_t n,
                                                              float* __restrict__ mean_frac, int* __restrict__ mean_int) {
  const int64_t s = blockIdx.x;
  const int16_t* p = x + s * in_stride;
  long long acc = 0;
  for (int64_t i = threadIdx.x; i < n; i += blockDim.x) acc += (long long)__ldg(p + i);
  __shared__ long long part[8];
#pragma unroll
  for (int off = 16; off > 0; off >>= 1) acc += __shfl_xor_sync(0xffffffffu, acc, off);
  if ((threadIdx.x & 31) == 0) part[threadIdx.x >> 5] = acc;
  __syncthreads();
  if (threadIdx.x == 0) {
    long long t = 0;
    for (int w = 0; w < 8; ++w) t += part[w];
    const double m = (double)t / (double)n;
    const int mi = (int)llrint(m);
    mean_int[s] = mi;
    mean_frac[s] = (float)(m - (double)mi);
  }
}
}

extern "C" int vadx_stream_mean_i16(const int16_t* d_audio, int64_t in_stride, int64_t n_samples, int64_t n_streams,
                                    float* d_mean_frac, int32_t* d_mean_int, void* stream) {
  StageTimer _timer(VADX_STAGE_PREP, (cudaStream_t)stream, "stream_mean_i16_kernel", 2.0 * n_streams * n_samples);
  VADX_REQUIRE(d_audio && d_mean_frac && d_mean_int && n_samples > 0 && in_stride >= n_samples && n_streams >= 0,
               "vadx_stream_mean_i16: bad argument");
  if (n_streams == 0) return VADX_OK;
  stream_mean_i16_kernel<<<(unsigned)n_streams, 256, 0, (cudaStream_t)stream>>>(d_audio, in_stride, n_samples, d_mean_frac,
                                                                                d_mean_int);
  return after_launch("vadx_stream_mean_i16");
}

extern "C" int vadx_stft_power_tc_i16(const int16_t* d_audio, int64_t in_stride, int64_t n_samples, int64_t n_streams,
                                      int n_frames, int hop, int n_taps, const void* d_img, int n_bins, float* d_power,
                                      int64_t ld_power, void* stream) {
  VADX_REQUIRE((int64_t)(n_frames - 1) * hop + n_taps <= n_samples,
               "vadx_stft_power_tc_i16: frames must lie inside the %lld samples of a stream", (long long)n_samples);
  return vadx_stft_power_tc_i16_ex(d_audio, in_stride, n_samples, n_streams, n_frames, hop, n_taps, d_img, n_bins, d_power,
                                   ld_power, 0, nullptr, nullptr, nullptr, 0, n_frames, 1.0f, VADX_TC_FMT_BF16, stream);
}

extern "C" int vadx_stft_power_tc_i16_ex(const int16_t* d_audio, int64_t in_stride, int64_t n_samples, int64_t n_streams,
                                         int n_frames, int hop, int n_taps, const void* d_img, int n_bins, float* d_power,
                                         int64_t ld_power, int pad_left, const float* d_mean_frac, const int32_t* d_mean_int,
                                         const float* d_dc_tables, int n_edge_lo, int t_edge_hi, float power_scale,
                                         int operand_format, void* stream) {
  const float* d_mean = d_mean_frac;
  VADX_REQUIRE(operand_format == VADX_TC_FMT_BF16 || (operand_format == VADX_TC_FMT_F16 && !d_mean_frac),
               "vadx_stft_power_tc_i16: fp16 operands cannot carry the mean-removed (17-bit) samples");
  VADX_REQUIRE((d_mean_frac == nullptr) == (d_mean_int == nullptr), "vadx_stft_power_tc_i16: mean needs both its parts");
  StageTimer _timer(VADX_STAGE_STFT, (cudaStream_t)stream, "stft_power_tc_kernel",
                    2.0 * n_streams * n_samples + 4.0 * n_streams * n_frames * n_bins,
                    2.0 * n_streams * n_frames * n_taps * 2.0 * n_bins);
  VADX_REQUIRE(d_audio && d_img && d_power, "vadx_stft_power_tc_i16: null pointer");
  VADX_REQUIRE(n_streams >= 0 && n_frames > 0 && hop > 0 && n_taps > 0 && n_bins > 0 && ld_power >= n_bins,
               "vadx_stft_power_tc_i16: bad shape");
  VADX_REQUIRE(in_stride >= n_samples && pad_left >= 0 && (pad_left % 8) == 0 && (n_samples % 8) == 0,
               "vadx_stft_power_tc_i16: stride shorter than the stream, or pad_left / n_samples not a multiple of 8");
  const bool leaves_stream = pad_left > 0 || (int64_t)(n_frames - 1) * hop - pad_left + n_taps > n_samples;
  VADX_REQUIRE(!(d_mean || leaves_stream) || (d_dc_tables && n_edge_lo >= 0 && t_edge_hi >= n_edge_lo && t_edge_hi <= n_frames),
               "vadx_stft_power_tc_i16: padded frames / DC removal need the tables of vadx_pack_stft_dc_tc");
  VADX_REQUIRE((hop % 16) == 0,
               "vadx_stft_power_tc_i16: hop %d is not a multiple of 16 samples (frames are read as shifted rows of 16-sample "
               "hop slices); use vadx_stft_power_f32", hop);
  VADX_REQUIRE((in_stride % 8) == 0 && aligned16(d_audio) && aligned16(d_img),
               "vadx_stft_power_tc_i16: stream stride must be a multiple of 8 samples, pointers 16-byte aligned");
  StftTcShape s = stft_tc_shape(n_taps, n_bins, hop);
  VADX_REQUIRE(s.ok, "vadx_stft_power_tc_i16: shape not supported");
  if (n_streams == 0) return VADX_OK;
  static PerDevice per_device;
  int n_sm = 148;
  VADX_TRY(per_device.ensure(&n_sm, [] {
    cudaError_t e = cudaSuccess;
    auto opt_in = [&](auto kern) {
      if (e == cudaSuccess) e = cudaFuncSetAttribute(kern, cudaFuncAttributeMaxDynamicSharedMemorySize, kTcSmemBudget);
    };
    opt_in(stft_power_tc_kernel<false, false>);
    opt_in(stft_power_tc_kernel<true, false>);
    opt_in(stft_power_tc_kernel<false, true>);
    opt_in(stft_power_tc_kernel<true, true>);
    return e;
  }));
  const StftTcRing ring = stft_tc_ring(s.n_k16, hop / 16);
  StftTcArgs g{};
  g.X = d_audio; g.in_stride = in_stride; g.L = n_samples; g.S = n_streams; g.n_frames = n_frames; g.hop = hop;
  g.h16 = hop / 16; g.n_q = ring.n_q; g.tq = n_frames + ring.n_q - 1; g.rows = ring.rows; g.slice_units = ring.slice_units;
  g.n_st = (int)ceil_div(g.h16, kStJ);
  g.Wimg = static_cast<const uint8_t*>(d_img); g.P = d_power; g.ldp = ld_power;
  g.n_bins = n_bins; g.kc = s.kc; g.n_k16 = s.n_k16;
  g.pad_left = pad_left; g.mean = d_mean; g.mean_int = d_mean_int; g.dc = d_dc_tables; g.power_scale = power_scale; g.n_edge_lo = n_edge_lo; g.t_edge_hi = t_edge_hi;
  g.vec_p = ((ld_power & 3) == 0) && aligned16(d_power);
  {
    static const int dbg = ab_env("VADX_TC_DEBUG", 0);
    g.debug = dbg;
  }
  static const int opt = ab_env("VADX_ST_OPT", 2);
  {
    static const int bl = ab_env("VADX_TC_BACKOFF_LD", 64);
    static const int be = ab_env("VADX_TC_BACKOFF_EPI", 256);
    g.backoff_ld = (unsigned)bl; g.backoff_epi = (unsigned)be;
  }
  g.stage_out = ((opt & 2) && g.vec_p && s.smem_bytes + s.stage_bytes <= (size_t)kTcSmemBudget) ? 1 : 0;
  const size_t smem = s.smem_bytes + (g.stage_out ? s.stage_bytes : 0);
  int64_t tiles = ceil_div(n_streams * g.tq, kTcBM);
  VADX_REQUIRE(tiles <= 0x7fffffffLL, "vadx_stft_power_tc_i16: too many rows");
  g.n_tiles = (int)tiles;
  int per = std::max(1, n_sm / s.n_ntiles);
  dim3 grid((unsigned)std::min<int64_t>(tiles, per), (unsigned)s.n_ntiles);
  const bool ex = leaves_stream || d_mean, f16 = operand_format == VADX_TC_FMT_F16;
  constexpr int kThreads = (kStLoaderWarps + 5) * 32;
  if (ex && f16) stft_power_tc_kernel<true, true><<<grid, kThreads, smem, (cudaStream_t)stream>>>(g);
  else if (ex) stft_power_tc_kernel<true, false><<<grid, kThreads, smem, (cudaStream_t)stream>>>(g);
  else if (f16) stft_power_tc_kernel<false, true><<<grid, kThreads, smem, (cudaStream_t)stream>>>(g);
  else stft_power_tc_kernel<false, false><<<grid, kThreads, smem, (cudaStream_t)stream>>>(g);
  return after_launch("vadx_stft_power_tc_i16");
}
```

### voice-activity-detection-vad-onnx_b200/csrc/tc_ptx.cuh

```cuda
#pragma once
#include "common.cuh"

namespace vadx {

constexpr int kTcBM = 128;
constexpr int kTcBK = 64;
constexpr int kTcTileBytes = kTcBM * 128;
constexpr int kTcSmemBudget = 227 * 1024;

__device__ __forceinline__ uint32_t smem_u32(const void* p) { return (uint32_t)__cvta_generic_to_shared(p); }

__device__ __forceinline__ void mbar_init(uint32_t bar, uint32_t count) {
  asm volatile("mbarrier.init.shared::cta.b64 [%0], %1;" ::"r"(bar), "r"(count));
}
__device__ __forceinline__ void mbar_arrive(uint32_t bar) {
  asm volatile("mbarrier.arrive.shared::cta.b64 _, [%0];" ::"r"(bar) : "memory");
}
__device__ __forceinline__ void mbar_expect_tx(uint32_t bar, uint32_t bytes) {
  asm volatile("mbarrier.arrive.expect_tx.shared::cta.b64 _, [%0], %1;" ::"r"(bar), "r"(bytes) : "memory");
}
__device__ __forceinline__ bool mbar_try_wait(uint32_t bar, uint32_t parity) {
  uint32_t ok;
  asm volatile(
      "{\n.reg .pred p;\nmbarrier.try_wait.parity.shared::cta.b64 p, [%1], %2;\nselp.u32 %0, 1, 0, p;\n}\n"
      : "=r"(ok)
      : "r"(bar), "r"(parity)
      : "memory");
  return ok != 0;
}
__device__ __forceinline__ void mbar_wait(uint32_t bar, uint32_t parity, unsigned backoff_ns = 0) {
  if (mbar_try_wait(bar, parity)) return;
  const long long t0 = clock64();
  while (!mbar_try_wait(bar, parity)) {
    if (backoff_ns) __nanosleep(backoff_ns);
    if (clock64() - t0 > 20000000000LL) __trap();
  }
}
__device__ __forceinline__ void fence_proxy_async() { asm volatile("fence.proxy.async.shared::cta;" ::: "memory"); }
__device__ __forceinline__ void tc_fence_before() { asm volatile("tcgen05.fence::before_thread_sync;" ::: "memory"); }
__device__ __forceinline__ void tc_fence_after() { asm volatile("tcgen05.fence::after_thread_sync;" ::: "memory"); }

__device__ __forceinline__ void bulk_g2s(uint32_t dst, const void* src, uint32_t bytes, uint32_t bar) {
  asm volatile("cp.async.bulk.shared::cluster.global.mbarrier::complete_tx::bytes [%0], [%1], %2, [%3];" ::"r"(dst),
               "l"(src), "r"(bytes), "r"(bar)
               : "memory");
}

__device__ __forceinline__ void bulk_s2g(void* dst, uint32_t src, uint32_t bytes) {
  asm volatile("cp.async.bulk.global.shared::cta.bulk_group [%0], [%1], %2;" ::"l"(dst), "r"(src), "r"(bytes) : "memory");
}

__device__ __forceinline__ uint64_t umma_desc_sw128(uint32_t smem_addr) {
  uint64_t d = 0;
  d |= (uint64_t)((smem_addr & 0x3FFFFu) >> 4);
  d |= (uint64_t)1 << 16;
  d |= (uint64_t)(1024 >> 4) << 32;
  d |= (uint64_t)1 << 46;
  d |= (uint64_t)2 << 61;
  return d;
}
__device__ __forceinline__ uint64_t umma_desc_noswz(uint32_t smem_addr, uint32_t lbo, uint32_t sbo) {
  uint64_t d = 0;
  d |= (uint64_t)((smem_addr & 0x3FFFFu) >> 4);
  d |= (uint64_t)((lbo >> 4) & 0x3FFFu) << 16;
  d |= (uint64_t)((sbo >> 4) & 0x3FFFu) << 32;
  d |= (uint64_t)1 << 46;
  return d;
}
__device__ __forceinline__ uint32_t umma_idesc_bf16(int n) {
  return (1u << 4) | (1u << 7) | (1u << 10) | ((uint32_t)(n >> 3) << 17) | ((uint32_t)(kTcBM >> 4) << 24);
}
__device__ __forceinline__ uint32_t umma_idesc_f16(int n) {
  return (1u << 4) | ((uint32_t)(n >> 3) << 17) | ((uint32_t)(kTcBM >> 4) << 24);
}
__device__ __forceinline__ void umma_bf16(uint32_t tmem_d, uint64_t adesc, uint64_t bdesc, uint32_t idesc,
                                          uint32_t accumulate) {
  asm volatile(
      "{\n.reg .pred p;\nsetp.ne.b32 p, %4, 0;\ntcgen05.mma.cta_group::1.kind::f16 [%0], %1, %2, %3, p;\n}\n" ::"r"(tmem_d),
      "l"(adesc), "l"(bdesc), "r"(idesc), "r"(accumulate)
      : "memory");
}
__device__ __forceinline__ void umma_k64(uint32_t tmem_d, uint64_t adesc, uint64_t bdesc, uint32_t idesc,
                                         uint32_t accumulate_first, int n_steps) {
  asm volatile(
      "{\n"
      ".reg .pred p0, pt, q1, q2, q3;\n"
      ".reg .b64 a1, a2, a3, b1, b2, b3;\n"
      "setp.ne.b32 p0, %4, 0;\n"
      "setp.eq.b32 pt, 0, 0;\n"
      "setp.gt.s32 q1, %5, 1;\n"
      "setp.gt.s32 q2, %5, 2;\n"
      "setp.gt.s32 q3, %5, 3;\n"
      "add.u64 a1, %1, 2;\n"
      "add.u64 a2, %1, 4;\n"
      "add.u64 a3, %1, 6;\n"
      "add.u64 b1, %2, 2;\n"
      "add.u64 b2, %2, 4;\n"
      "add.u64 b3, %2, 6;\n"
      "tcgen05.mma.cta_group::1.kind::f16 [%0], %1, %2, %3, p0;\n"
      "@q1 tcgen05.mma.cta_group::1.kind::f16 [%0], a1, b1, %3, pt;\n"
      "@q2 tcgen05.mma.cta_group::1.kind::f16 [%0], a2, b2, %3, pt;\n"
      "@q3 tcgen05.mma.cta_group::1.kind::f16 [%0], a3, b3, %3, pt;\n"
      "}\n" ::"r"(tmem_d),
      "l"(adesc), "l"(bdesc), "r"(idesc), "r"(accumulate_first), "r"(n_steps)
      : "memory");
}
__device__ __forceinline__ void umma_x2(uint32_t tmem_d, uint64_t adesc0, uint64_t adesc1, uint64_t bdesc, uint32_t idesc,
                                        uint32_t accumulate_first) {
  asm volatile(
      "{\n.reg .pred p, pt;\n"
      "setp.ne.b32 p, %5, 0;\n"
      "setp.eq.b32 pt, 0, 0;\n"
      "tcgen05.mma.cta_group::1.kind::f16 [%0], %1, %3, %4, p;\n"
      "tcgen05.mma.cta_group::1.kind::f16 [%0], %2, %3, %4, pt;\n"
      "}\n" ::"r"(tmem_d),
      "l"(adesc0), "l"(adesc1), "l"(bdesc), "r"(idesc), "r"(accumulate_first)
      : "memory");
}
__device__ __forceinline__ void umma_split_x3(uint32_t tmem_d, uint64_t a, uint32_t a_step, uint32_t a_lo, uint64_t b0,
                                              uint64_t b1, uint64_t b2, uint32_t idesc, uint32_t accumulate_first,
                                              int n_pairs, uint32_t lo_on) {
  asm volatile(
      "{\n"
      ".reg .pred p0, pt, q1, q2, l0, l1, l2;\n"
      ".reg .b64 st, lo, a0h, a1, a1h, a2, a2h;\n"
      "setp.ne.b32 p0, %7, 0;\n"
      "setp.eq.b32 pt, 0, 0;\n"
      "setp.gt.s32 q1, %8, 1;\n"
      "setp.gt.s32 q2, %8, 2;\n"
      "setp.ne.b32 l0, %9, 0;\n"
      "and.pred l1, l0, q1;\n"
      "and.pred l2, l0, q2;\n"
      "cvt.u64.u32 st, %2;\n"
      "cvt.u64.u32 lo, %3;\n"
      "add.u64 a0h, %1, lo;\n"
      "add.u64 a1, %1, st;\n"
      "add.u64 a1h, a1, lo;\n"
      "add.u64 a2, a1, st;\n"
      "add.u64 a2h, a2, lo;\n"
      "tcgen05.mma.cta_group::1.kind::f16 [%0], %1, %4, %6, p0;\n"
      "@l0 tcgen05.mma.cta_group::1.kind::f16 [%0], a0h, %4, %6, pt;\n"
      "@q1 tcgen05.mma.cta_group::1.kind::f16 [%0], a1, %5, %6, pt;\n"
      "@l1 tcgen05.mma.cta_group::1.kind::f16 [%0], a1h, %5, %6, pt;\n"
      "@q2 tcgen05.mma.cta_group::1.kind::f16 [%0], a2, %10, %6, pt;\n"
      "@l2 tcgen05.mma.cta_group::1.kind::f16 [%0], a2h, %10, %6, pt;\n"
      "}\n" ::"r"(tmem_d),
      "l"(a), "r"(a_step), "r"(a_lo), "l"(b0), "l"(b1), "r"(idesc), "r"(accumulate_first), "r"(n_pairs), "r"(lo_on),
      "l"(b2)
      : "memory");
}
__device__ __forceinline__ void umma_commit(uint32_t bar) {
  asm volatile("tcgen05.commit.cta_group::1.mbarrier::arrive::one.shared::cluster.b64 [%0];" ::"r"(bar) : "memory");
}
__device__ __forceinline__ void tmem_ld16(uint32_t taddr, float* v) {
  uint32_t r[16];
  asm volatile(
      "tcgen05.ld.sync.aligned.32x32b.x16.b32 {%0,%1,%2,%3,%4,%5,%6,%7,%8,%9,%10,%11,%12,%13,%14,%15}, [%16];"
      : "=r"(r[0]), "=r"(r[1]), "=r"(r[2]), "=r"(r[3]), "=r"(r[4]), "=r"(r[5]), "=r"(r[6]), "=r"(r[7]), "=r"(r[8]),
        "=r"(r[9]), "=r"(r[10]), "=r"(r[11]), "=r"(r[12]), "=r"(r[13]), "=r"(r[14]), "=r"(r[15])
      : "r"(taddr));
  asm volatile("tcgen05.wait::ld.sync.aligned;" ::: "memory");
#pragma unroll
  for (int i = 0; i < 16; ++i) v[i] = __uint_as_float(r[i]);
}

__device__ __forceinline__ void tmem_ld8_issue(uint32_t taddr, uint32_t* r) {
  asm volatile("tcgen05.ld.sync.aligned.32x32b.x8.b32 {%0,%1,%2,%3,%4,%5,%6,%7}, [%8];"
               : "=r"(r[0]), "=r"(r[1]), "=r"(r[2]), "=r"(r[3]), "=r"(r[4]), "=r"(r[5]), "=r"(r[6]), "=r"(r[7])
               : "r"(taddr));
}
__device__ __forceinline__ void tmem_ld8_finish(uint32_t* r) {
  asm volatile("tcgen05.wait::ld.sync.aligned;"
               : "+r"(r[0]), "+r"(r[1]), "+r"(r[2]), "+r"(r[3]), "+r"(r[4]), "+r"(r[5]), "+r"(r[6]), "+r"(r[7])
               :
               : "memory");
}

__device__ __forceinline__ void tmem_ld8(uint32_t taddr, float* v) {
  uint32_t r[8];
  asm volatile("tcgen05.ld.sync.aligned.32x32b.x8.b32 {%0,%1,%2,%3,%4,%5,%6,%7}, [%8];"
               : "=r"(r[0]), "=r"(r[1]), "=r"(r[2]), "=r"(r[3]), "=r"(r[4]), "=r"(r[5]), "=r"(r[6]), "=r"(r[7])
               : "r"(taddr));
  asm volatile("tcgen05.wait::ld.sync.aligned;" ::: "memory");
#pragma unroll
  for (int i = 0; i < 8; ++i) v[i] = __uint_as_float(r[i]);
}

__device__ __forceinline__ void l2_prefetch(const void* p, uint32_t bytes) {
  asm volatile("cp.async.bulk.prefetch.L2.global [%0], %1;" ::"l"(p), "r"(bytes) : "memory");
}

__device__ __forceinline__ void ldg256_nc(const float* p, float4& a, float4& b) {
  asm volatile("ld.global.nc.v8.f32 {%0,%1,%2,%3,%4,%5,%6,%7}, [%8];"
               : "=f"(a.x), "=f"(a.y), "=f"(a.z), "=f"(a.w), "=f"(b.x), "=f"(b.y), "=f"(b.z), "=f"(b.w)
               : "l"(p));
}

__device__ __forceinline__ void tmem_ld32(uint32_t taddr, float* v) {
  uint32_t r[32];
  asm volatile(
      "tcgen05.ld.sync.aligned.32x32b.x32.b32 "
      "{%0,%1,%2,%3,%4,%5,%6,%7,%8,%9,%10,%11,%12,%13,%14,%15,%16,%17,%18,%19,%20,%21,%22,%23,%24,%25,%26,%27,%28,%29,%30,%31}, [%32];"
      : "=r"(r[0]), "=r"(r[1]), "=r"(r[2]), "=r"(r[3]), "=r"(r[4]), "=r"(r[5]), "=r"(r[6]), "=r"(r[7]), "=r"(r[8]),
        "=r"(r[9]), "=r"(r[10]), "=r"(r[11]), "=r"(r[12]), "=r"(r[13]), "=r"(r[14]), "=r"(r[15]), "=r"(r[16]),
        "=r"(r[17]), "=r"(r[18]), "=r"(r[19]), "=r"(r[20]), "=r"(r[21]), "=r"(r[22]), "=r"(r[23]), "=r"(r[24]),
        "=r"(r[25]), "=r"(r[26]), "=r"(r[27]), "=r"(r[28]), "=r"(r[29]), "=r"(r[30]), "=r"(r[31])
      : "r"(taddr));
  asm volatile("tcgen05.wait::ld.sync.aligned;" ::: "memory");
#pragma unroll
  for (int i = 0; i < 32; ++i) v[i] = __uint_as_float(r[i]);
}

__device__ __forceinline__ void split2(float a, float b, uint32_t& hi, uint32_t& lo) {
  asm("cvt.rn.bf16x2.f32 %0, %1, %2;" : "=r"(hi) : "f"(b), "f"(a));
  float ah = __uint_as_float(hi << 16), bh = __uint_as_float(hi & 0xffff0000u);
  float al = a - ah, bl = b - bh;
  asm("cvt.rn.bf16x2.f32 %0, %1, %2;" : "=r"(lo) : "f"(bl), "f"(al));
}


static inline uint16_t bf16_rn_host(float f) {
  uint32_t u;
  memcpy(&u, &f, 4);
  if ((u & 0x7f800000u) == 0x7f800000u) return (uint16_t)(u >> 16);
  u += 0x7fffu + ((u >> 16) & 1u);
  return (uint16_t)(u >> 16);
}
static inline float bf16_to_f_host(uint16_t h) {
  uint32_t u = (uint32_t)h << 16;
  float f;
  memcpy(&f, &u, 4);
  return f;
}
static inline uint16_t f16_rn_host(float f) {
  uint32_t u;
  memcpy(&u, &f, 4);
  const uint32_t sign = (u >> 16) & 0x8000u;
  const int32_t exp = (int32_t)((u >> 23) & 0xffu) - 127 + 15;
  uint32_t man = u & 0x7fffffu;
  if (((u >> 23) & 0xffu) == 0xffu) return (uint16_t)(sign | 0x7c00u | (man ? 0x200u : 0u));
  if (exp >= 31) return (uint16_t)(sign | 0x7c00u);
  if (exp <= 0) {
    if (exp < -10) return (uint16_t)sign;
    man |= 0x800000u;
    const int shift = 14 - exp;
    uint32_t h = man >> shift;
    const uint32_t rem = man & ((1u << shift) - 1u), halfway = 1u << (shift - 1);
    if (rem > halfway || (rem == halfway && (h & 1u))) ++h;
    return (uint16_t)(sign | h);
  }
  uint32_t h = ((uint32_t)exp << 10) | (man >> 13);
  const uint32_t rem = man & 0x1fffu;
  if (rem > 0x1000u || (rem == 0x1000u && (h & 1u))) ++h;
  return (uint16_t)(sign | h);
}
static inline float f16_to_f_host(uint16_t h) {
  const uint32_t sign = (uint32_t)(h & 0x8000u) << 16;
  const uint32_t exp = (h >> 10) & 0x1fu, man = h & 0x3ffu;
  float f;
  if (exp == 0) {
    f = ldexpf((float)man, -24);
    uint32_t u;
    memcpy(&u, &f, 4);
    u |= sign;
    memcpy(&f, &u, 4);
    return f;
  }
  const uint32_t u = exp == 31 ? (sign | 0x7f800000u | (man << 13)) : (sign | ((exp - 15 + 127) << 23) | (man << 13));
  memcpy(&f, &u, 4);
  return f;
}
static inline size_t sw128_offset(int r, int kk) {
  return (size_t)(r / 8) * 1024 + (size_t)(r % 8) * 128 + (size_t)(((kk / 8) ^ (r % 8)) * 16) + (size_t)(kk % 8) * 2;
}

}
```

### voice-activity-detection-vad-onnx_b200/lib.py

```python
from __future__ import annotations

import ctypes as C
import os

_HERE = os.path.dirname(os.path.abspath(__file__))
LIB_PATH = os.path.join(_HERE, "libvadx.so")

DT_I16, DT_F32, DT_I32 = 0, 1, 2
ACT_NONE, ACT_RELU, ACT_SIGMOID, ACT_SOFTMAX, ACT_RES_FIRST = 0, 1, 2, 3, 16
FLOOR_CLAMP, FLOOR_ADD = 0, 1
PREEMPH_NONE, PREEMPH_ZERO_HISTORY, PREEMPH_KEEP_FIRST = 0, 1, 2

_ERRORS = {-1: ValueError, -2: RuntimeError, -3: RuntimeError, -4: KeyError, -5: MemoryError}


class PostCfg(C.Structure):
    _fields_ = [("smooth_window", C.c_int32), ("threshold", C.c_float), ("min_speech_frame", C.c_int32),
                ("max_speech_frame", C.c_int32), ("min_silence_frame", C.c_int32),
                ("merge_silence_frame", C.c_int32), ("extend_speech_frame", C.c_int32)]


class StreamPostCfg(C.Structure):
    _fields_ = [("smooth_window", C.c_int32), ("threshold", C.c_float), ("pad_start_frame", C.c_int32),
                ("min_speech_frame", C.c_int32), ("max_speech_frame", C.c_int32), ("min_silence_frame", C.c_int32)]


_i64, _i32, _f32, _vp, _sz = C.c_int64, C.c_int, C.c_float, C.c_void_p, C.c_size_t

SIGNATURES = {
    "vadx_abi_version": (C.c_int, []),
    "vadx_last_error": (C.c_char_p, []),
    "vadx_device_count": (C.c_int, []),
    "vadx_launch_count": (C.c_uint64, []),
    "vadx_profile_enable": (C.c_int, [_i32]),
    "vadx_profile_collect": (C.c_int, [C.POINTER(C.c_double), C.POINTER(C.c_uint64), _i32]),
    "vadx_profile_collect_kernels": (C.c_int, [_vp, _i32, C.POINTER(C.c_int)]),
    "vadx_prep_audio": (C.c_int, [_vp, _i32, _i64, _i64, _i64, _f32, _i32, _i32, _f32, _i64, _vp, _i64, _vp]),
    "vadx_stft_power_f32": (C.c_int, [_vp, _i64, _i64, _i32, _i32, _i32, _vp, _i32, _i32, _vp, _i64, _vp]),
    "vadx_stft_tc_supported": (C.c_int, [_i32, _i32]),
    "vadx_pack_stft_basis_tc": (C.c_int, [_vp, _i32, _i32, _i32, C.c_double, C.c_double, _vp, _sz, C.POINTER(_sz)]),
    "vadx_stft_power_tc_i16": (C.c_int, [_vp, _i64, _i64, _i64, _i32, _i32, _i32, _vp, _i32, _vp, _i64, _vp]),
    "vadx_pack_stft_dc_tc": (C.c_int, [_vp, _i32, _i32, _i32, C.c_double, C.c_double, _i64, _i32, _i32, _i32, _vp, _sz,
                                       C.POINTER(_sz), C.POINTER(C.c_int), C.POINTER(C.c_int)]),
    "vadx_stream_mean_i16": (C.c_int, [_vp, _i64, _i64, _i64, _vp, _vp, _vp]),
    "vadx_stft_power_tc_i16_ex": (C.c_int, [_vp, _i64, _i64, _i64, _i32, _i32, _i32, _vp, _i32, _vp, _i64, _i32, _vp, _vp, _vp,
                                            _i32, _i32, _f32, _i32, _vp]),
    "vadx_pack_stft_basis_tc_fmt": (C.c_int, [_vp, _i32, _i32, _i32, C.c_double, C.c_double, _i32, _vp, _sz, C.POINTER(_sz)]),
    "vadx_mel_log_f32": (C.c_int, [_vp, _i64, _i64, _i32, _i32, _vp, _vp, _vp, _i32, _i32, _f32, _vp, _i64, _vp]),
    "vadx_linear_f32": (C.c_int, [_vp, _i64, _vp, _i32, _vp, _vp, _i64, _vp, _i64, _i64, _i32, _i32, _i32, _vp]),
    "vadx_tc_supported": (C.c_int, [_i32, _i32]),
    "vadx_pack_weight_tc": (C.c_int, [_vp, _i32, _i32, _vp, _sz, C.POINTER(_sz)]),
    "vadx_linear_tc_f32": (C.c_int, [_vp, _i64, _vp, _vp, _vp, _i64, _vp, _i64, _i64, _i32, _i32, _i32, _vp]),
    "vadx_fc2_memory_stages_stream_bytes": (C.c_size_t, [_i32, _i32]),
    "vadx_fc2_memory_stages_supported": (C.c_int, [_i32, _i32, _i32, _i32, _i32, _i32, _i32]),
    "vadx_linear_tc_stream_stages_f32": (C.c_int, [_vp, _vp, _vp, _vp, _i64, _i32, _i32, _i32, _i32, _vp]),
    "vadx_fc2_memory_stages_f32": (C.c_int, [_vp, _i32, _vp, _vp, _i32, _vp, _i32, _vp, _i32, _vp, _vp, _i64, _i32, _vp]),
    "vadx_depthwise_conv1d_f32": (C.c_int, [_vp, _i64, _vp, _i32, _i32, _i32, _i32, _vp, _i64, _i64, _i32, _i32, _i32, _vp]),
    "vadx_linear_head_tc_f32": (C.c_int, [_vp, _i64, _vp, _vp, _i64, _i32, _i32, _i32, _vp, _f32, _vp, _vp]),
    "vadx_fsmn_memory_f32": (C.c_int, [_vp, _i64, _vp, _i32, _i32, _vp, _i32, _i32, _vp, _i64, _vp, _i64, _i64,
                                       _i32, _i32, _vp, _vp, _vp]),
    "vadx_lfr_cmvn_f32": (C.c_int, [_vp, _i64, _vp, _vp, _vp, _i64, _i64, _i32, _i32, _i32, _i32, _vp]),
    "vadx_softmax_class0_f32": (C.c_int, [_vp, _i64, _i64, _i32, _vp, _vp]),
    "vadx_frame_energy_log10_f32": (C.c_int, [_vp, _i64, _i64, _i64, _i32, _i32, _i32, _i32, _f32, _f32, _vp, _vp]),
    "vadx_fsmn_gate": (C.c_int, [_vp, _vp, _vp, _f32, _f32, _i64, _i32, _vp, _vp, _vp]),
    "vadx_cfb_front_supported": (C.c_int, [_i32, _i32, _i32]),
    "vadx_cfb_front_f32": (C.c_int, [_vp, _i64, _i32, _i32, _i32, _vp, _vp, _vp, _vp, _vp, _vp, _vp, _vp, _vp, _vp, C.c_float, _vp, _vp, _vp]),
    "vadx_layernorm_perm_f32": (C.c_int, [_vp, _i64, _i32, _i32, _i32, _i32, _i32, _i32, _vp, _vp, _i32, C.c_float, _vp, _i64, _i32, _vp]),
    "vadx_ceps_cmul_t_f32": (C.c_int, [_vp, _vp, _vp, _i64, _i32, _i32, _vp]),
    "vadx_add_transposed_f32": (C.c_int, [_vp, _i64, _vp, _vp, _i64, _i32, _i32, _vp]),
    "vadx_lstm_recurrence_supported": (C.c_int, [_i32]),
    "vadx_lstm_recurrence_f32": (C.c_int, [_vp, _i64, _i64, _i64, _vp, _i64, _i64, _i64, _vp, _i64, _i32, _i32, _i32, _i32, _vp]),
    "vadx_affine_f32": (C.c_int, [_vp, C.c_float, C.c_float, _vp, _i64, _vp]),
    "vadx_reflect_windows_f32": (C.c_int, [_vp, _i64, _i64, _i32, _i64, _i32, _i32, _vp, _vp]),
    "vadx_silero_lstm_windows_f32": (C.c_int, [_vp, _vp, _i32, _vp, _vp, _vp, C.c_float, _vp, _i64, _i32, _i32, _vp]),
    "vadx_stft_mag_compact_f32": (C.c_int, [_vp, _i64, _i64, _i32, _i32, _i32, _vp, _vp]),
    "vadx_gather_windows_i16": (C.c_int, [_vp, _i64, _i64, _i32, _i64, _i64, _vp, _vp]),
    "vadx_fsmn_gate_hysteresis_windows": (C.c_int, [_vp, _vp, _i64, _i32, _i32, C.c_float, C.c_float, _i32, C.c_double, C.c_double,
                                                    _vp, _vp, _vp, _vp, _vp, _vp, _i64, _vp, C.c_float, _vp]),
    "vadx_lookahead_hysteresis": (C.c_int, [_vp, _i32, _i64, _i64, _i32, _i32, C.c_double, C.c_double, _i32, _vp, _vp,
                                            _vp, _i64, _vp, _vp, _f32, _vp]),
    "vadx_runs_to_segments": (C.c_int, [_vp, _i64, _vp, _i64, _vp, _vp, _i32, _vp]),
    "vadx_reflect_window_f32": (C.c_int, [_vp, _i64, _i64, _i32, _i32, _vp, _vp]),
    "vadx_sqrt_inplace_f32": (C.c_int, [_vp, _i64, _vp]),
    "vadx_lstm_cell_f32": (C.c_int, [_vp, _vp, _vp, _vp, _vp, _i64, _i32, _vp]),
    "vadx_silero_timestamps": (C.c_int, [_vp, _i64, _vp, _vp, _i64, C.c_double, C.c_double, C.c_double, C.c_double,
                                         C.c_double, C.c_double, _i32, _i32, _vp, _vp, _i32, _vp]),
    "vadx_stft_complex_f32": (C.c_int, [_vp, _i64, _i64, _i32, _i32, _i32, _vp, _i32, _i32, _vp, _i64, _vp]),
    "vadx_permute4_f32": (C.c_int, [_vp, _vp, _i64, _i64, _i64, _i64, _i32, _i32, _i32, _i32, _vp]),
    "vadx_layernorm_f32": (C.c_int, [_vp, _i64, _i32, _vp, _vp, _f32, _vp, _vp]),
    "vadx_lstm_seq_f32": (C.c_int, [_vp, _i64, _i64, _i64, _vp, _i64, _i64, _i64, _vp, _vp, _vp, _vp, _i64, _i32, _i32,
                                    _i32, _i32, _i32, _vp]),
    "vadx_ew2_f32": (C.c_int, [_i32, _vp, _i64, _vp, _i64, _vp, _i64, _vp, _i64, _i64, _i32, _f32, _vp]),
    "vadx_ceps_cmul_f32": (C.c_int, [_vp, _vp, _vp, _i64, _i32, _vp]),
    "vadx_im2col_f3_f32": (C.c_int, [_vp, _vp, _i64, _i32, _i32, _vp]),
    "vadx_alpha_x4_f32": (C.c_int, [_vp, _vp, _i64, _i32, _i32, _i32, _f32, _f32, _f32, _vp, _f32, _vp, _vp, _vp]),
    "vadx_alpha_x4_const_f32": (C.c_int, [_vp, _vp, _vp, _i32, _i64, _i32, _i32, _i32, _f32, _f32, _f32, _vp, _f32, _vp, _vp,
                                          _vp]),
    "vadx_istft_ola_f32": (C.c_int, [_vp, _i64, _i64, _i32, _i32, _i32, _vp, _i32, _vp, _i64, _vp]),
    "vadx_postprocess_frames": (C.c_int, [_vp, _i64, _vp, _i64, _i32, C.POINTER(PostCfg), _vp, _vp, _vp, _i32, _vp]),
    "vadx_resample_out_len": (C.c_int64, [_i64, C.c_double]),
    "vadx_resample_linear_f32": (C.c_int, [_vp, _i64, _i64, _i64, C.c_double, _vp, _i64, _i64, _vp]),
    "vadx_ingest_out_frames": (C.c_int64, [_i64, _i32, _i32]),
    "vadx_ingest_pcm16": (C.c_int, [_vp, _i64, _vp, _i64, _i64, _i32, _i32, _i32, _vp, _i64, _vp, _vp]),
    "vadx_stream_post_state_words": (C.c_int, [_i32]),
    "vadx_stream_postprocess": (C.c_int, [_vp, _i64, _vp, _i64, _i32, C.POINTER(StreamPostCfg), _vp, _vp, _vp, _i32, _vp,
                                          _vp]),
    "vadx_stream_serve_zero_tail": (C.c_int, [_vp, _i64, _vp, _i64, _i32, _i32, _vp]),
    "vadx_stream_serve_step": (C.c_int, [_vp, _i64, _i32, _vp, _vp, _i64, _i32, _i32, _i32, C.POINTER(StreamPostCfg), _vp,
                                         _vp, _vp, _i32, _i64, _vp, _vp, _vp, _vp, _vp, _vp, _sz, C.POINTER(_sz), _vp]),
    "vadx_silero_serve_load": (C.c_int, [_vp, _vp, _i64, _i32, _vp, _vp]),
    "vadx_silero_serve_step": (C.c_int, [_vp, _i64, _vp, _vp, _i64, _i32, C.c_double, C.c_double, _vp, _vp, _vp, _vp, _vp,
                                         _vp, _vp, _vp, _vp, _vp, _sz, C.POINTER(_sz), _vp]),
    "vadx_create": (C.c_int, [C.c_char_p, C.POINTER(C.c_int32), _i32, C.POINTER(_vp)]),
    "vadx_destroy": (None, [_vp]),
    "vadx_set_tensor": (C.c_int, [_vp, C.c_char_p, _vp, _i32, C.POINTER(_i64), _i32]),
    "vadx_set_scalar": (C.c_int, [_vp, C.c_char_p, C.c_double]),
    "vadx_workspace_bytes": (C.c_int, [_vp, _i64, _i64, C.POINTER(_sz)]),
    "vadx_output_frames": (C.c_int, [_vp, _i64, C.POINTER(C.c_int32)]),
    "vadx_forward": (C.c_int, [_vp, C.POINTER(_vp), C.POINTER(_vp), C.POINTER(_vp), _i64, _i64, _vp, _sz, _vp]),
}

_lib = None


def load() -> C.CDLL:
    global _lib
    if _lib is not None:
        return _lib
    if not os.path.exists(LIB_PATH):
        raise RuntimeError(
            f"{LIB_PATH} is missing: build it with `python -c 'import __graft_entry__ as g; g.build()'` "
            "(vadx has no CPU or PyTorch fallback)")
    lib = C.CDLL(LIB_PATH)
    for name, (res, args) in SIGNATURES.items():
        fn = getattr(lib, name)
        fn.restype = res
        fn.argtypes = args
    if lib.vadx_abi_version() != 1:
        raise RuntimeError(f"libvadx ABI {lib.vadx_abi_version()} != 1; rebuild the library")
    _lib = lib
    return lib


STAGES = ("prep", "stft", "mel", "linear", "memory", "head", "postproc")


def profile_enable(on: bool) -> None:
    check(load().vadx_profile_enable(1 if on else 0))


def profile_collect() -> dict:
    ms = (C.c_double * len(STAGES))()
    calls = (C.c_uint64 * len(STAGES))()
    check(load().vadx_profile_collect(ms, calls, len(STAGES)))
    return {n: (ms[i], int(calls[i])) for i, n in enumerate(STAGES)}


class _KernelStat(C.Structure):
    _fields_ = [("name", C.c_char_p), ("ms", C.c_double), ("calls", C.c_uint64), ("bytes", C.c_double), ("flops", C.c_double)]


def profile_collect_kernels() -> dict:
    n = C.c_int(0)
    check(load().vadx_profile_collect_kernels(None, 0, C.byref(n)))
    if n.value == 0:
        return {}
    buf = (_KernelStat * n.value)()
    check(load().vadx_profile_collect_kernels(C.cast(buf, C.c_void_p), n.value, C.byref(n)))
    return {buf[i].name.decode(): {"ms": buf[i].ms, "calls": int(buf[i].calls), "bytes": buf[i].bytes, "flops": buf[i].flops}
            for i in range(n.value)}


def check(rc: int) -> None:
    if rc == 0:
        return
    msg = load().vadx_last_error().decode("utf-8", "replace")
    raise _ERRORS.get(rc, RuntimeError)(f"libvadx: {msg} (code {rc})")


def require_device() -> None:
    if load().vadx_device_count() < 1:
        raise RuntimeError("libvadx: no CUDA device visible; vadx has no CPU path")


def pack_weight_tc(w):
    import numpy as np
    w = np.ascontiguousarray(w, np.float32)
    n_out, n_in = w.shape
    nbytes = C.c_size_t()
    check(load().vadx_pack_weight_tc(w.ctypes.data, n_out, n_in, None, 0, C.byref(nbytes)))
    img = np.zeros(nbytes.value, np.uint8)
    check(load().vadx_pack_weight_tc(w.ctypes.data, n_out, n_in, img.ctypes.data, img.nbytes, C.byref(nbytes)))
    return img


TC_FMT_BF16, TC_FMT_F16 = 0, 1


def pack_stft_basis_tc(basis, n_bins: int, preemph: float, scale: float, fmt: int = TC_FMT_BF16):
    import numpy as np
    basis = np.ascontiguousarray(basis, np.float32)
    n_taps, ld = basis.shape
    nbytes = C.c_size_t()
    check(load().vadx_pack_stft_basis_tc_fmt(basis.ctypes.data, ld, n_taps, n_bins, preemph, scale, fmt, None, 0,
                                             C.byref(nbytes)))
    img = np.zeros(nbytes.value, np.uint8)
    check(load().vadx_pack_stft_basis_tc_fmt(basis.ctypes.data, ld, n_taps, n_bins, preemph, scale, fmt, img.ctypes.data,
                                             img.nbytes, C.byref(nbytes)))
    return img


def pack_stft_dc_tc(basis, n_bins: int, preemph: float, scale: float, n_samples: int, hop: int, pad_left: int,
                    n_frames: int):
    import numpy as np
    basis = np.ascontiguousarray(basis, np.float32)
    n_taps, ld = basis.shape
    n, lo, hi = C.c_size_t(), C.c_int(), C.c_int()
    check(load().vadx_pack_stft_dc_tc(basis.ctypes.data, ld, n_taps, n_bins, preemph, scale, n_samples, hop, pad_left,
                                      n_frames, None, 0, C.byref(n), C.byref(lo), C.byref(hi)))
    tab = np.zeros(n.value, np.float32)
    check(load().vadx_pack_stft_dc_tc(basis.ctypes.data, ld, n_taps, n_bins, preemph, scale, n_samples, hop, pad_left,
                                      n_frames, tab.ctypes.data, tab.size, C.byref(n), C.byref(lo), C.byref(hi)))
    return tab, lo.value, hi.value


def ptr(t) -> int:
    if t is None:
        return 0
    if hasattr(t, "data_ptr"):
        return t.data_ptr()
    return t.ctypes.data


def stream_ptr(stream=None) -> int:
    import torch
    s = stream if stream is not None else torch.cuda.current_stream()
    return s.cuda_stream
```

Baseline: 372.4.

## Add int8 tensor-core STFT path with split-byte audio and scaled basis

Adds an i8 operand format for the tensor-core STFT power kernel. Int16 audio is split into high and low signed/unsigned bytes, and the basis is quantized to three int8 terms with per-column scales. The pieces are recombined in the epilogue before squaring. FireRed now selects this format by default, falling back to fp16 when hop, padding or DC removal do not fit. The change trades more MMA issues and a heavier epilogue for the higher int8 throughput and half-size operands. It also halves the loader warps and adds precision risk from quantizing the basis.

```diff
diff --git a/include/vadx.h b/include/vadx.h
--- a/include/vadx.h
+++ b/include/vadx.h
@@ -76,7 +76,7 @@
                               int64_t ld_power, int pad_left, const float* d_mean_frac, const int32_t* d_mean_int,
                               const float* d_dc_tables, int n_edge_lo, int t_edge_hi, float power_scale,
                               int operand_format, void* stream);
-enum { VADX_TC_FMT_BF16 = 0, VADX_TC_FMT_F16 = 1 };
+enum { VADX_TC_FMT_BF16 = 0, VADX_TC_FMT_F16 = 1, VADX_TC_FMT_I8 = 2 };
 int vadx_pack_stft_basis_tc_fmt(const float* h_basis, int ld_basis, int n_taps, int n_bins, double preemph, double scale,
                                 int operand_format, void* h_img, size_t img_capacity, size_t* img_bytes);
 
diff --git a/voice-activity-detection-vad-onnx_b200/csrc/model.cu b/voice-activity-detection-vad-onnx_b200/csrc/model.cu
--- a/voice-activity-detection-vad-onnx_b200/csrc/model.cu
+++ b/voice-activity-detection-vad-onnx_b200/csrc/model.cu
@@ -18,7 +18,7 @@
 
 static Frontend firered_frontend(const vadx_model* m, const FireRedHP& h) {
   return Frontend{h, (int)m->scalar("derived.bins_used", (double)h.n_bins()), 0, 1.0f, false, VADX_PREEMPH_ZERO_HISTORY,
-                  VADX_TC_FMT_F16, VADX_FLOOR_CLAMP, (float)m->scalar("frontend.log_floor", 1e-7), frontend_rate_scale(m),
+                  VADX_TC_FMT_I8, VADX_FLOOR_CLAMP, (float)m->scalar("frontend.log_floor", 1e-7), frontend_rate_scale(m),
                   false};
 }
 
diff --git a/voice-activity-detection-vad-onnx_b200/csrc/model.hpp b/voice-activity-detection-vad-onnx_b200/csrc/model.hpp
--- a/voice-activity-detection-vad-onnx_b200/csrc/model.hpp
+++ b/voice-activity-detection-vad-onnx_b200/csrc/model.hpp
@@ -259,6 +259,9 @@
   double rate_scale;
   bool keep_signal;
 
+  int tc_image_format() const {
+    return tc_format == VADX_TC_FMT_I8 && ((g.hop % 32) != 0 || pad_left != 0 || remove_dc) ? VADX_TC_FMT_F16 : tc_format;
+  }
   int finalize(vadx_model* m) const;
   int run(vadx_model* m, const int16_t* audio, int64_t S, int64_t L, int T, const FrontendBufs& b, cudaStream_t st) const;
 };
@@ -274,10 +277,11 @@
     const double preemph = m->scalar("frontend.preemph", 0.97);
     const float* hb = m->find("frontend.basis")->f32();
     size_t bytes = 0;
-    VADX_TRY(vadx_pack_stft_basis_tc_fmt(hb, g.ld_basis(), g.n_taps(), n_bins, preemph, 1.0, tc_format, nullptr, 0, &bytes));
+    VADX_TRY(vadx_pack_stft_basis_tc_fmt(hb, g.ld_basis(), g.n_taps(), n_bins, preemph, 1.0, tc_image_format(), nullptr, 0,
+                                         &bytes));
     std::vector<uint8_t> img(bytes);
-    VADX_TRY(vadx_pack_stft_basis_tc_fmt(hb, g.ld_basis(), g.n_taps(), n_bins, preemph, 1.0, tc_format, img.data(), img.size(),
-                                         &bytes));
+    VADX_TRY(vadx_pack_stft_basis_tc_fmt(hb, g.ld_basis(), g.n_taps(), n_bins, preemph, 1.0, tc_image_format(), img.data(),
+                                         img.size(), &bytes));
     VADX_TRY(m->upload("frontend.basis#TC", img.data(), img.size()));
   }
   VADX_TRY(m->upload_raw("frontend.mel_start", g.n_mels, VADX_DT_I32));
@@ -311,7 +315,9 @@
     VADX_TRY(vadx_stft_power_f32(b.sig2, Lp, S, T, g.hop, g.n_taps(), m->d<float>("frontend.basis"), g.ld_basis(), n_bins,
                                  b.power, g.ld_power(), st));
   } else {
-    const bool tc = stft_img && (L % 8) == 0 && (g.hop % 16) == 0 && (pad_left % 8) == 0 && aligned16(audio);
+    const bool frames_inside = (int64_t)(T - 1) * g.hop + g.n_taps() <= L;
+    const bool tc = stft_img && (L % 8) == 0 && (g.hop % 16) == 0 && (pad_left % 8) == 0 && aligned16(audio) &&
+                    (frames_inside || tc_image_format() != VADX_TC_FMT_I8);
     if (keep_signal || !tc)
       VADX_TRY(vadx_prep_audio(audio, VADX_DT_I16, S, L, L, in_scale, remove_dc, pre, preemph, pad_left, b.sig, Lp, st));
     if (tc) {
@@ -339,7 +345,7 @@
       if (remove_dc) VADX_TRY(vadx_stream_mean_i16(audio, L, L, S, b.mean, b.mean_int, st));
       VADX_TRY(vadx_stft_power_tc_i16_ex(audio, L, L, S, T, g.hop, g.n_taps(), stft_img, n_bins, b.power, g.ld_power(), pad_left,
                                          remove_dc ? b.mean : nullptr, remove_dc ? b.mean_int : nullptr, dc, lo, hi,
-                                         in_scale * in_scale, tc_format, st));
+                                         in_scale * in_scale, tc_image_format(), st));
     } else {
       VADX_TRY(vadx_stft_power_f32(b.sig, Lp, S, T, g.hop, g.n_taps(), m->d<float>("frontend.basis"), g.ld_basis(), n_bins,
                                    b.power, g.ld_power(), st));
diff --git a/voice-activity-detection-vad-onnx_b200/csrc/stft_tc.cu b/voice-activity-detection-vad-onnx_b200/csrc/stft_tc.cu
--- a/voice-activity-detection-vad-onnx_b200/csrc/stft_tc.cu
+++ b/voice-activity-detection-vad-onnx_b200/csrc/stft_tc.cu
@@ -8,8 +8,14 @@
 constexpr int kStJ = 2;
 constexpr int kStSlices = 2 * kStJ;
 constexpr int kStStages = 3;
-constexpr int kStLoaderWarps = 16;
+constexpr int stft_loader_warps(int fmt) { return fmt == VADX_TC_FMT_I8 ? 8 : 16; }
+constexpr int kStI8NPad = 64;
+constexpr int kStI8Terms = 3;
+constexpr int kStI8QMax = 127 * (65536 + 256 + 1);
+constexpr int stft_npad(int fmt) { return fmt == VADX_TC_FMT_I8 ? kStI8NPad : kStNPad; }
+constexpr int stft_terms(int fmt) { return fmt == VADX_TC_FMT_I8 ? kStI8Terms : kStTerms; }
 constexpr int kStOutLd = 44;
+constexpr int stft_threads(int fmt) { return (stft_loader_warps(fmt) + 5) * 32; }
 
 struct StftTcArgs {
   const int16_t* X;
@@ -24,6 +30,7 @@
   int slice_units;
   int n_st;
   const uint8_t* Wimg;
+  const float* col_scale;
   float* P;
   int64_t ldp;
   int n_bins, kc, n_k16, n_tiles, vec_p;
@@ -71,13 +78,17 @@
   hi = fmaf(__uint_as_float(0x4B000000u | h), 256.0f, -(8388608.0f + 256.0f) * 256.0f);
 }
 
-template <bool EX, bool F16>
-__global__ void __launch_bounds__((kStLoaderWarps + 5) * 32, 1) stft_power_tc_kernel(const StftTcArgs g) {
+template <bool EX, int FMT>
+__global__ void __launch_bounds__(stft_threads(FMT), 1) stft_power_tc_kernel(const StftTcArgs g) {
+  constexpr bool F16 = FMT == VADX_TC_FMT_F16, I8 = FMT == VADX_TC_FMT_I8;
+  constexpr int kStLoaderWarps = stft_loader_warps(FMT);
   constexpr int kStEpiWarp0 = kStLoaderWarps, kStMmaWarp = kStLoaderWarps + 4;
+  constexpr int kNPad = stft_npad(FMT), kTerms = stft_terms(FMT);
+  static_assert(!(I8 && EX), "the i8 variant reads frames inside the stream only");
   extern __shared__ __align__(1024) uint8_t smem_raw[];
   uint8_t* w_smem = smem_raw;
-  const uint32_t img_bytes = kStNPad * 128u;
-  const int w_bytes = g.kc * kStTerms * (int)img_bytes;
+  const uint32_t img_bytes = kNPad * 128u;
+  const int w_bytes = g.kc * kTerms * (int)img_bytes;
   uint8_t* a_smem = w_smem + w_bytes;
   const uint32_t slice_bytes = (uint32_t)g.slice_units * 16u;
   const uint32_t term_bytes = kStSlices * slice_bytes;
@@ -93,7 +104,7 @@
   auto tfull_bar = [&](int b) { return bar0 + 8u * (8 + b); };
   auto tempty_bar = [&](int b) { return bar0 + 8u * (10 + b); };
   const uint32_t wbar = bar0 + 8u * 12;
-  constexpr int kAccN = 2 * kStNPad;
+  constexpr int kAccN = (I8 ? 4 : 2) * kNPad;
   constexpr uint32_t kTmemCols = 512;
 
   if (threadIdx.x == 0) {
@@ -124,12 +135,14 @@
     if (lane == 0) {
       mbar_expect_tx(wbar, (uint32_t)w_bytes);
       const uint8_t* src = g.Wimg + (size_t)ntile * w_bytes;
-      for (int t = 0; t < g.kc * kStTerms; ++t) bulk_g2s(smem_u32(w_smem) + t * img_bytes, src + (size_t)t * img_bytes, img_bytes, wbar);
+      for (int t = 0; t < g.kc * kTerms; ++t) bulk_g2s(smem_u32(w_smem) + t * img_bytes, src + (size_t)t * img_bytes, img_bytes, wbar);
       mbar_wait(wbar, 0);
       const uint32_t idesc = F16 ? umma_idesc_f16(kAccN) : umma_idesc_bf16(kAccN);
+      constexpr uint32_t kIdescHi = umma_idesc_i8(3 * kNPad, true), kIdescLo = umma_idesc_i8(3 * kNPad, false);
+      constexpr uint32_t kIdescLoB0 = umma_idesc_i8(kNPad, false), kIdescLoTop = umma_idesc_i8(2 * kNPad, false);
       const uint64_t dw = umma_desc_sw128(smem_u32(w_smem));
       const uint64_t da0 = umma_desc_noswz(smem_u32(a_smem), slice_bytes, 128u);
-      const uint32_t chunk_units = (kStTerms * img_bytes) >> 4, lo_units = term_bytes >> 4, stage_units = stage_bytes >> 4;
+      const uint32_t chunk_units = (kTerms * img_bytes) >> 4, lo_units = term_bytes >> 4, stage_units = stage_bytes >> 4;
       const uint32_t col_units = (2u * slice_bytes) >> 4;
       const int h16 = g.h16, n_k16 = g.n_k16;
       const uint32_t lo_on = (g.debug & 4) ? 0u : 1u;
@@ -153,7 +166,20 @@
             const int j = st * kStJ + jj;
             if (j >= h16) break;
             const uint64_t da_j = da_st + (uint64_t)jj * col_units;
-            if (kBurst) {
+            if constexpr (I8) {
+              int q0 = 0, k = j;
+              if (k == 0) {
+                umma_i8_first(d_tmem, d_tmem + kNPad, d_tmem + 3 * kNPad, da_j, lo_units, dw, (2 * img_bytes) >> 4, kIdescHi,
+                              kIdescLoB0, kIdescLoTop, lo_on);
+                q0 = 1;
+                k = h16;
+              }
+              for (; k < n_k16; q0 += 3, k += 3 * h16) {
+                const int n_pairs = 1 + (k + h16 < n_k16 ? 1 : 0) + (k + 2 * h16 < n_k16 ? 1 : 0);
+                umma_i8_x3(d_tmem, d_tmem + kNPad, da_j + (uint64_t)q0, 1u, lo_units, b_desc(k), b_desc(k + h16), b_desc(k + 2 * h16),
+                           kIdescHi, kIdescLo, n_pairs, lo_on);
+              }
+            } else if (kBurst) {
               for (int q0 = 0, k = j; k < n_k16; q0 += 3, k += 3 * h16) {
                 const int n_pairs = 1 + (k + h16 < n_k16 ? 1 : 0) + (k + 2 * h16 < n_k16 ? 1 : 0);
                 umma_split_x3(d_tmem, da_j + (uint64_t)q0, 1u, lo_units, b_desc(k), b_desc(k + h16), b_desc(k + 2 * h16),
@@ -175,7 +201,8 @@
     }
   } else if (warp < kStLoaderWarps) {
     constexpr int kRowsPerPass = kStLoaderWarps * 32 / kStSlices;
-    constexpr int kPasses = 2;
+    constexpr int kPasses = 256 / kRowsPerPass;
+    constexpr int kRaw = I8 ? 2 : 1;
     const int t = threadIdx.x;
     const int sl = t % kStSlices;
     const int r_in = t / kStSlices;
@@ -206,14 +233,16 @@
       }
       const int grp = q.st * kStSlices + sl;
 #pragma unroll
-      for (int pass = 0; pass < kPasses; ++pass) {
-        const int i0 = h0_n[pass] + 8 * grp;
+      for (int pass = 0; pass < kPasses; ++pass)
+#pragma unroll
+      for (int h = 0; h < kRaw; ++h) {
+        const int i0 = h0_n[pass] + 8 * (kRaw * grp + h);
         uint4 v = make_uint4(0u, 0u, 0u, 0u);
         if (((rok_n >> pass) & 1u) && grp < n_groups && i0 >= 0 && i0 + 7 < g.L) {
           v = __ldg(reinterpret_cast<const uint4*>(xs_n[pass] + i0));
           msk |= 1u << pass;
         }
-        raw[pass] = v;
+        raw[pass * kRaw + h] = v;
       }
     };
     int stage = 0;
@@ -239,9 +268,15 @@
       for (int pass = 0; pass < kPasses; ++pass) {
         const int r = pass * kRowsPerPass + r_in;
         if (r >= g.rows) break;
-        const uint32_t wds[4] = {raw[pass].x, raw[pass].y, raw[pass].z, raw[pass].w};
+        const uint32_t wds[4] = {raw[pass * kRaw].x, raw[pass * kRaw].y, raw[pass * kRaw].z, raw[pass * kRaw].w};
         uint32_t hi[4], lo[4];
-        if (EX && g.mean_int) {
+        if constexpr (I8) {
+          const uint4 v = raw[pass * kRaw + 1];
+          hi[0] = __byte_perm(wds[0], wds[1], 0x7531); lo[0] = __byte_perm(wds[0], wds[1], 0x6420);
+          hi[1] = __byte_perm(wds[2], wds[3], 0x7531); lo[1] = __byte_perm(wds[2], wds[3], 0x6420);
+          hi[2] = __byte_perm(v.x, v.y, 0x7531);       lo[2] = __byte_perm(v.x, v.y, 0x6420);
+          hi[3] = __byte_perm(v.z, v.w, 0x7531);       lo[3] = __byte_perm(v.z, v.w, 0x6420);
+        } else if (EX && g.mean_int) {
           const int mi = ((msk >> pass) & 1u) ? mi_c[pass] : 0;
 #pragma unroll
           for (int j = 0; j < 4; ++j) {
@@ -270,8 +305,8 @@
       if (lane == 0) mbar_arrive(full_bar(stage));
       if (++stage == kStStages) { stage = 0; phase ^= 1u; }
     };
-    constexpr int kStBufs = EX ? 4 : 6;
-    uint4 bufs[kStBufs][kPasses];
+    constexpr int kStBufs = I8 ? 2 : (EX ? 4 : 6);
+    uint4 bufs[kStBufs][kPasses * kRaw];
     uint32_t msks[kStBufs];
 #pragma unroll
     for (int i = 0; i < kStBufs; ++i) msks[i] = 0u;
@@ -291,7 +326,7 @@
   } else {
     const int q = warp - kStEpiWarp0;
     int it = 0;
-    const int f0 = ntile * (kStNPad / 2);
+    const int f0 = ntile * (kNPad / 2);
     for (int tile = blockIdx.x; tile < g.n_tiles; tile += gridDim.x, ++it) {
       const int b = it & 1;
       const uint32_t use = (uint32_t)(it >> 1);
@@ -320,12 +355,25 @@
         }
       }
 #pragma unroll
-      for (int c0 = 0; c0 < kStNPad; c0 += 16) {
+      for (int c0 = 0; c0 < kNPad; c0 += 16) {
         float v[16], v2[16];
         tmem_ld16(taddr + (uint32_t)c0, v);
-        tmem_ld16(taddr + (uint32_t)(kStNPad + c0), v2);
-#pragma unroll
-        for (int j = 0; j < 16; ++j) v[j] += v2[j];
+        tmem_ld16(taddr + (uint32_t)(kNPad + c0), v2);
+        if constexpr (I8) {
+#pragma unroll
+          for (int j = 0; j < 16; ++j)
+            v[j] = fmaf(__int2float_rn(__float_as_int(v[j])), 16777216.0f, __int2float_rn(__float_as_int(v2[j])) * 65536.0f);
+          tmem_ld16(taddr + (uint32_t)(2 * kNPad + c0), v2);
+#pragma unroll
+          for (int j = 0; j < 16; ++j) v[j] = fmaf(__int2float_rn(__float_as_int(v2[j])), 256.0f, v[j]);
+          tmem_ld16(taddr + (uint32_t)(3 * kNPad + c0), v2);
+          const float* cs = g.col_scale + ntile * kNPad + c0;
+#pragma unroll
+          for (int j = 0; j < 16; ++j) v[j] = (v[j] + __int2float_rn(__float_as_int(v2[j]))) * __ldg(cs + j);
+        } else {
+#pragma unroll
+          for (int j = 0; j < 16; ++j) v[j] += v2[j];
+        }
         if (!row_ok || (g.debug & 1)) continue;
         if (EX && dc_row) {
 #pragma unroll
@@ -357,7 +405,27 @@
       __syncwarp();
       if (lane == 0) mbar_arrive(tempty_bar(b));
       if (g.stage_out && !(g.debug & 1)) {
-        constexpr int kC4 = kStNPad / 8;
+        constexpr int kC4 = kNPad / 8;
+        if constexpr (I8) {
+#pragma unroll 1
+          for (int itr = 0; itr < kC4; ++itr) {
+            const int idx = itr * 32 + lane;
+            const int r = idx / kC4, c4 = idx - r * kC4;
+            const long long grow = __shfl_sync(0xffffffffu, (long long)row, r);
+            const int fbin = f0 + c4 * 4;
+            if (grow >= 0 && fbin < g.n_bins) {
+              const float4 val = *reinterpret_cast<const float4*>(my_out + r * kStOutLd + c4 * 4);
+              float* out = g.P + grow * g.ldp + fbin;
+              if (fbin + 3 < g.n_bins) {
+                *reinterpret_cast<float4*>(out) = val;
+              } else {
+                out[0] = val.x;
+                if (fbin + 1 < g.n_bins) out[1] = val.y;
+                if (fbin + 2 < g.n_bins) out[2] = val.z;
+              }
+            }
+          }
+        } else {
 #pragma unroll
         for (int itr = 0; itr < kC4; ++itr) {
           const int idx = itr * 32 + lane;
@@ -376,6 +444,7 @@
             }
           }
         }
+        }
         __syncwarp();
       }
     }
@@ -406,15 +475,16 @@
   size_t tile_bytes, img_bytes, smem_bytes, stage_bytes;
   bool ok;
 };
-StftTcShape stft_tc_shape(int n_taps, int n_bins, int hop = 16) {
+StftTcShape stft_tc_shape(int n_taps, int n_bins, int hop = 16, int fmt = VADX_TC_FMT_BF16) {
   StftTcShape s{};
   const int k_used = n_taps + kStLead;
-  s.kc = (int)ceil_div(k_used, kTcBK);
-  s.n_k16 = (int)ceil_div(k_used, 16);
-  s.n_ntiles = (int)ceil_div(2 * n_bins, kStNPad);
-  s.tile_bytes = (size_t)s.kc * kStTerms * kStNPad * 128;
-  s.img_bytes = s.tile_bytes * s.n_ntiles;
-  s.smem_bytes = s.tile_bytes + stft_tc_ring(s.n_k16, std::max(1, hop / 16)).bytes + 16 * 8;
+  const int k_step = fmt == VADX_TC_FMT_I8 ? 32 : 16;
+  s.kc = (int)ceil_div(k_used, fmt == VADX_TC_FMT_I8 ? 128 : kTcBK);
+  s.n_k16 = (int)ceil_div(k_used, k_step);
+  s.n_ntiles = (int)ceil_div(2 * n_bins, stft_npad(fmt));
+  s.tile_bytes = (size_t)s.kc * stft_terms(fmt) * stft_npad(fmt) * 128;
+  s.img_bytes = s.tile_bytes * s.n_ntiles + (fmt == VADX_TC_FMT_I8 ? (size_t)s.n_ntiles * kStI8NPad * sizeof(float) : 0);
+  s.smem_bytes = s.tile_bytes + stft_tc_ring(s.n_k16, std::max(1, hop / k_step)).bytes + 16 * 8;
   s.stage_bytes = (size_t)4 * 32 * kStOutLd * sizeof(float);
   s.ok = s.smem_bytes <= (size_t)kTcSmemBudget;
   return s;
@@ -437,10 +507,10 @@
                                            size_t* img_bytes) {
   VADX_REQUIRE(h_basis && img_bytes && n_taps > 0 && n_bins > 0 && ld_basis >= 2 * n_bins,
                "vadx_pack_stft_basis_tc: bad argument");
-  VADX_REQUIRE(operand_format == VADX_TC_FMT_BF16 || operand_format == VADX_TC_FMT_F16, "vadx_pack_stft_basis_tc: operand format %d",
-               operand_format);
+  VADX_REQUIRE(operand_format == VADX_TC_FMT_BF16 || operand_format == VADX_TC_FMT_F16 || operand_format == VADX_TC_FMT_I8,
+               "vadx_pack_stft_basis_tc: operand format %d", operand_format);
   const bool f16 = operand_format == VADX_TC_FMT_F16;
-  StftTcShape s = stft_tc_shape(n_taps, n_bins);
+  StftTcShape s = stft_tc_shape(n_taps, n_bins, 16, operand_format);
   VADX_REQUIRE(s.ok, "vadx_pack_stft_basis_tc: %d taps x %d bins does not fit the tensor-core DFT", n_taps, n_bins);
   *img_bytes = s.img_bytes;
   if (!h_img) return VADX_OK;
@@ -449,14 +519,41 @@
   memset(img, 0, s.img_bytes);
   const int n_cols = 2 * n_bins;
   const size_t term = (size_t)kStNPad * 128;
+  auto folded = [&](int k, int col) {
+    const int n0 = k - kStLead, n1 = k - kStLead + 1;
+    double v = 0.0;
+    if (n0 >= 0 && n0 < n_taps) v += (double)h_basis[(size_t)n0 * ld_basis + col];
+    if (n1 >= 0 && n1 < n_taps) v -= preemph * (double)h_basis[(size_t)n1 * ld_basis + col];
+    return v * scale;
+  };
+  if (operand_format == VADX_TC_FMT_I8) {
+    const size_t term8 = (size_t)kStI8NPad * 128;
+    float* col_scale = reinterpret_cast<float*>(img + s.tile_bytes * s.n_ntiles);
+    for (int f = 0; f < n_bins; ++f) {
+      double m = 0.0;
+      for (int col = 2 * f; col < 2 * f + 2; ++col)
+        for (int k = 0; k < n_taps + kStLead; ++k) m = std::max(m, std::fabs(folded(k, col)));
+      const int e = m > 0.0 ? std::min(60, std::max(-60, (int)std::floor(std::log2((double)kStI8QMax / m)))) : 0;
+      for (int col = 2 * f; col < 2 * f + 2; ++col) {
+        const int nt = col / kStI8NPad, r = col % kStI8NPad;
+        col_scale[col] = std::ldexp(1.0f, -e);
+        for (int k = 0; k < n_taps + kStLead; ++k) {
+          long long q = std::llround(std::ldexp(folded(k, col), e));
+          uint8_t* base = img + (size_t)nt * s.tile_bytes + (size_t)((k / 128) * kStI8Terms) * term8 + sw128_offset_b8(r, k % 128);
+          for (int t = kStI8Terms - 1; t >= 0; --t) {
+            const long long d = t > 0 ? ((q + 128) & 255) - 128 : q;
+            base[(size_t)t * term8] = (uint8_t)(int8_t)d;
+            q = (q - d) / 256;
+          }
+        }
+      }
+    }
+    return VADX_OK;
+  }
   for (int col = 0; col < n_cols; ++col) {
     const int nt = col / kStNPad, r = col % kStNPad;
     for (int k = 0; k < n_taps + kStLead; ++k) {
-      const int n0 = k - kStLead, n1 = k - kStLead + 1;
-      double v = 0.0;
-      if (n0 >= 0 && n0 < n_taps) v += (double)h_basis[(size_t)n0 * ld_basis + col];
-      if (n1 >= 0 && n1 < n_taps) v -= preemph * (double)h_basis[(size_t)n1 * ld_basis + col];
-      v *= scale;
+      const double v = folded(k, col);
       const float f = (float)v;
       const uint16_t b0 = f16 ? f16_rn_host(f) : bf16_rn_host(f);
       const float r1 = (float)(v - (double)(f16 ? f16_to_f_host(b0) : bf16_to_f_host(b0)));
@@ -563,8 +660,11 @@
                                          const float* d_dc_tables, int n_edge_lo, int t_edge_hi, float power_scale,
                                          int operand_format, void* stream) {
   const float* d_mean = d_mean_frac;
-  VADX_REQUIRE(operand_format == VADX_TC_FMT_BF16 || (operand_format == VADX_TC_FMT_F16 && !d_mean_frac),
-               "vadx_stft_power_tc_i16: fp16 operands cannot carry the mean-removed (17-bit) samples");
+  VADX_REQUIRE(operand_format == VADX_TC_FMT_BF16 ||
+                   ((operand_format == VADX_TC_FMT_F16 || operand_format == VADX_TC_FMT_I8) && !d_mean_frac),
+               "vadx_stft_power_tc_i16: operand format %d (fp16 and i8 operands cannot carry the mean-removed 17-bit samples)",
+               operand_format);
+  const bool i8 = operand_format == VADX_TC_FMT_I8;
   VADX_REQUIRE((d_mean_frac == nullptr) == (d_mean_int == nullptr), "vadx_stft_power_tc_i16: mean needs both its parts");
   StageTimer _timer(VADX_STAGE_STFT, (cudaStream_t)stream, "stft_power_tc_kernel",
                     2.0 * n_streams * n_samples + 4.0 * n_streams * n_frames * n_bins,
@@ -580,10 +680,17 @@
   VADX_REQUIRE((hop % 16) == 0,
                "vadx_stft_power_tc_i16: hop %d is not a multiple of 16 samples (frames are read as shifted rows of 16-sample "
                "hop slices); use vadx_stft_power_f32", hop);
+  VADX_REQUIRE(!i8 || !leaves_stream,
+               "vadx_stft_power_tc_i16: i8 operands read frames inside the stream only (no centre pad, no tail); use an fp16 "
+               "or bf16 image");
+  VADX_REQUIRE(!i8 || (hop % 32) == 0,
+               "vadx_stft_power_tc_i16: hop %d is not a multiple of 32 samples (i8 operands read 32-sample hop slices); use "
+               "an fp16 or bf16 image", hop);
   VADX_REQUIRE((in_stride % 8) == 0 && aligned16(d_audio) && aligned16(d_img),
                "vadx_stft_power_tc_i16: stream stride must be a multiple of 8 samples, pointers 16-byte aligned");
-  StftTcShape s = stft_tc_shape(n_taps, n_bins, hop);
+  StftTcShape s = stft_tc_shape(n_taps, n_bins, hop, operand_format);
   VADX_REQUIRE(s.ok, "vadx_stft_power_tc_i16: shape not supported");
+  const int k_step = i8 ? 32 : 16;
   if (n_streams == 0) return VADX_OK;
   static PerDevice per_device;
   int n_sm = 148;
@@ -592,18 +699,21 @@
     auto opt_in = [&](auto kern) {
       if (e == cudaSuccess) e = cudaFuncSetAttribute(kern, cudaFuncAttributeMaxDynamicSharedMemorySize, kTcSmemBudget);
     };
-    opt_in(stft_power_tc_kernel<false, false>);
-    opt_in(stft_power_tc_kernel<true, false>);
-    opt_in(stft_power_tc_kernel<false, true>);
-    opt_in(stft_power_tc_kernel<true, true>);
+    opt_in(stft_power_tc_kernel<false, VADX_TC_FMT_BF16>);
+    opt_in(stft_power_tc_kernel<true, VADX_TC_FMT_BF16>);
+    opt_in(stft_power_tc_kernel<false, VADX_TC_FMT_F16>);
+    opt_in(stft_power_tc_kernel<true, VADX_TC_FMT_F16>);
+    opt_in(stft_power_tc_kernel<false, VADX_TC_FMT_I8>);
     return e;
   }));
-  const StftTcRing ring = stft_tc_ring(s.n_k16, hop / 16);
+  const StftTcRing ring = stft_tc_ring(s.n_k16, hop / k_step);
   StftTcArgs g{};
   g.X = d_audio; g.in_stride = in_stride; g.L = n_samples; g.S = n_streams; g.n_frames = n_frames; g.hop = hop;
-  g.h16 = hop / 16; g.n_q = ring.n_q; g.tq = n_frames + ring.n_q - 1; g.rows = ring.rows; g.slice_units = ring.slice_units;
+  g.h16 = hop / k_step; g.n_q = ring.n_q; g.tq = n_frames + ring.n_q - 1; g.rows = ring.rows; g.slice_units = ring.slice_units;
   g.n_st = (int)ceil_div(g.h16, kStJ);
-  g.Wimg = static_cast<const uint8_t*>(d_img); g.P = d_power; g.ldp = ld_power;
+  g.Wimg = static_cast<const uint8_t*>(d_img);
+  g.col_scale = i8 ? reinterpret_cast<const float*>(g.Wimg + s.tile_bytes * s.n_ntiles) : nullptr;
+  g.P = d_power; g.ldp = ld_power;
   g.n_bins = n_bins; g.kc = s.kc; g.n_k16 = s.n_k16;
   g.pad_left = pad_left; g.mean = d_mean; g.mean_int = d_mean_int; g.dc = d_dc_tables; g.power_scale = power_scale; g.n_edge_lo = n_edge_lo; g.t_edge_hi = t_edge_hi;
   g.vec_p = ((ld_power & 3) == 0) && aligned16(d_power);
@@ -625,10 +735,12 @@
   int per = std::max(1, n_sm / s.n_ntiles);
   dim3 grid((unsigned)std::min<int64_t>(tiles, per), (unsigned)s.n_ntiles);
   const bool ex = leaves_stream || d_mean, f16 = operand_format == VADX_TC_FMT_F16;
-  constexpr int kThreads = (kStLoaderWarps + 5) * 32;
-  if (ex && f16) stft_power_tc_kernel<true, true><<<grid, kThreads, smem, (cudaStream_t)stream>>>(g);
-  else if (ex) stft_power_tc_kernel<true, false><<<grid, kThreads, smem, (cudaStream_t)stream>>>(g);
-  else if (f16) stft_power_tc_kernel<false, true><<<grid, kThreads, smem, (cudaStream_t)stream>>>(g);
-  else stft_power_tc_kernel<false, false><<<grid, kThreads, smem, (cudaStream_t)stream>>>(g);
+  constexpr int kThreads = stft_threads(VADX_TC_FMT_BF16), kThreadsI8 = stft_threads(VADX_TC_FMT_I8);
+  const cudaStream_t cs = (cudaStream_t)stream;
+  if (i8) stft_power_tc_kernel<false, VADX_TC_FMT_I8><<<grid, kThreadsI8, smem, cs>>>(g);
+  else if (ex && f16) stft_power_tc_kernel<true, VADX_TC_FMT_F16><<<grid, kThreads, smem, cs>>>(g);
+  else if (ex) stft_power_tc_kernel<true, VADX_TC_FMT_BF16><<<grid, kThreads, smem, cs>>>(g);
+  else if (f16) stft_power_tc_kernel<false, VADX_TC_FMT_F16><<<grid, kThreads, smem, cs>>>(g);
+  else stft_power_tc_kernel<false, VADX_TC_FMT_BF16><<<grid, kThreads, smem, cs>>>(g);
   return after_launch("vadx_stft_power_tc_i16");
 }
diff --git a/voice-activity-detection-vad-onnx_b200/csrc/tc_ptx.cuh b/voice-activity-detection-vad-onnx_b200/csrc/tc_ptx.cuh
--- a/voice-activity-detection-vad-onnx_b200/csrc/tc_ptx.cuh
+++ b/voice-activity-detection-vad-onnx_b200/csrc/tc_ptx.cuh
@@ -72,6 +72,9 @@
 }
 __device__ __forceinline__ uint32_t umma_idesc_f16(int n) {
   return (1u << 4) | ((uint32_t)(n >> 3) << 17) | ((uint32_t)(kTcBM >> 4) << 24);
+}
+__host__ __device__ constexpr uint32_t umma_idesc_i8(int n, bool a_signed) {
+  return (2u << 4) | ((a_signed ? 1u : 0u) << 7) | (1u << 10) | ((uint32_t)(n >> 3) << 17) | ((uint32_t)(kTcBM >> 4) << 24);
 }
 __device__ __forceinline__ void umma_bf16(uint32_t tmem_d, uint64_t adesc, uint64_t bdesc, uint32_t idesc,
                                           uint32_t accumulate) {
@@ -149,6 +152,57 @@
       "l"(b2)
       : "memory");
 }
+__device__ __forceinline__ void umma_i8_x3(uint32_t tmem_d, uint32_t tmem_d_lo, uint64_t a, uint32_t a_step, uint32_t a_lo,
+                                           uint64_t b0, uint64_t b1, uint64_t b2, uint32_t idesc_hi, uint32_t idesc_lo,
+                                           int n_pairs, uint32_t lo_on) {
+  asm volatile(
+      "{\n"
+      ".reg .pred pt, q1, q2, l0, l1, l2;\n"
+      ".reg .b64 st, lo, a0h, a1, a1h, a2, a2h;\n"
+      "setp.eq.b32 pt, 0, 0;\n"
+      "setp.gt.s32 q1, %9, 1;\n"
+      "setp.gt.s32 q2, %9, 2;\n"
+      "setp.ne.b32 l0, %10, 0;\n"
+      "and.pred l1, l0, q1;\n"
+      "and.pred l2, l0, q2;\n"
+      "cvt.u64.u32 st, %3;\n"
+      "cvt.u64.u32 lo, %4;\n"
+      "add.u64 a0h, %2, lo;\n"
+      "add.u64 a1, %2, st;\n"
+      "add.u64 a1h, a1, lo;\n"
+      "add.u64 a2, a1, st;\n"
+      "add.u64 a2h, a2, lo;\n"
+      "tcgen05.mma.cta_group::1.kind::i8 [%0], %2, %5, %7, pt;\n"
+      "@l0 tcgen05.mma.cta_group::1.kind::i8 [%1], a0h, %5, %8, pt;\n"
+      "@q1 tcgen05.mma.cta_group::1.kind::i8 [%0], a1, %6, %7, pt;\n"
+      "@l1 tcgen05.mma.cta_group::1.kind::i8 [%1], a1h, %6, %8, pt;\n"
+      "@q2 tcgen05.mma.cta_group::1.kind::i8 [%0], a2, %11, %7, pt;\n"
+      "@l2 tcgen05.mma.cta_group::1.kind::i8 [%1], a2h, %11, %8, pt;\n"
+      "}\n" ::"r"(tmem_d), "r"(tmem_d_lo),
+      "l"(a), "r"(a_step), "r"(a_lo), "l"(b0), "l"(b1), "r"(idesc_hi), "r"(idesc_lo), "r"(n_pairs), "r"(lo_on), "l"(b2)
+      : "memory");
+}
+__device__ __forceinline__ void umma_i8_first(uint32_t tmem_d, uint32_t tmem_d_lo, uint32_t tmem_d_b0, uint64_t a,
+                                              uint32_t a_lo, uint64_t b, uint32_t b_b0_units, uint32_t idesc_hi,
+                                              uint32_t idesc_lo_b0, uint32_t idesc_lo_top, uint32_t lo_on) {
+  asm volatile(
+      "{\n"
+      ".reg .pred pf, pt, l0;\n"
+      ".reg .b64 ah, bl;\n"
+      "setp.ne.b32 pf, 0, 0;\n"
+      "setp.eq.b32 pt, 0, 0;\n"
+      "setp.ne.b32 l0, %10, 0;\n"
+      "cvt.u64.u32 ah, %4;\n"
+      "add.u64 ah, %3, ah;\n"
+      "cvt.u64.u32 bl, %6;\n"
+      "add.u64 bl, %5, bl;\n"
+      "tcgen05.mma.cta_group::1.kind::i8 [%0], %3, %5, %7, pf;\n"
+      "@l0 tcgen05.mma.cta_group::1.kind::i8 [%2], ah, bl, %8, pf;\n"
+      "@l0 tcgen05.mma.cta_group::1.kind::i8 [%1], ah, %5, %9, pt;\n"
+      "}\n" ::"r"(tmem_d), "r"(tmem_d_lo), "r"(tmem_d_b0),
+      "l"(a), "r"(a_lo), "l"(b), "r"(b_b0_units), "r"(idesc_hi), "r"(idesc_lo_b0), "r"(idesc_lo_top), "r"(lo_on)
+      : "memory");
+}
 __device__ __forceinline__ void umma_commit(uint32_t bar) {
   asm volatile("tcgen05.commit.cta_group::1.mbarrier::arrive::one.shared::cluster.b64 [%0];" ::"r"(bar) : "memory");
 }
@@ -273,5 +327,8 @@
 static inline size_t sw128_offset(int r, int kk) {
   return (size_t)(r / 8) * 1024 + (size_t)(r % 8) * 128 + (size_t)(((kk / 8) ^ (r % 8)) * 16) + (size_t)(kk % 8) * 2;
 }
-
-}
+static inline size_t sw128_offset_b8(int r, int kk) {
+  return (size_t)(r / 8) * 1024 + (size_t)(r % 8) * 128 + (size_t)(((kk / 16) ^ (r % 8)) * 16) + (size_t)(kk % 16);
+}
+
+}
diff --git a/voice-activity-detection-vad-onnx_b200/lib.py b/voice-activity-detection-vad-onnx_b200/lib.py
--- a/voice-activity-detection-vad-onnx_b200/lib.py
+++ b/voice-activity-detection-vad-onnx_b200/lib.py
@@ -194,7 +194,7 @@
     return img
 
 
-TC_FMT_BF16, TC_FMT_F16 = 0, 1
+TC_FMT_BF16, TC_FMT_F16, TC_FMT_I8 = 0, 1, 2
 
 
 def pack_stft_basis_tc(basis, n_bins: int, preemph: float, scale: float, fmt: int = TC_FMT_BF16):
```

Measured after the change: 378.2, median of 6. +1.6%, better.
